# EI-CoreBioinformatics/portcullis

Hardware: AMD Instinct MI355X
Metric: junc_reads_per_sec (higher is better)
Workload: dtype int32; 1 GPU; BASELINE configs[2]: synthetic 199999998 paired-end 150-bp reads, 25 contigs of GRCh38 lengths (3088286401 bp), 249999 junctions, orientation FR; reads_total=199999998, junctions_total=249999, contigs=25, reads_rank0=199999998, pairs_rank0=66692850

## Files before the change

### portcullis_amd/csrc/pjb_api.hip

```cpp
#include "pjb_host.hip.h"
#include "pjb_kernels.hip.h"
#include "pjb_chain.hip.h"
#include "pjb_flight.hip.h"

extern "C" {

namespace {
std::mutex g_host_mu;
std::map<void *, size_t> g_host_registered;
}
void *pjb_host_alloc(size_t bytes) {
    if (bytes >= ((size_t)8 << 20)) {
        const size_t huge = (size_t)2 << 20, len = (bytes + huge - 1) & ~(huge - 1);
        void *p = mmap(nullptr, len, PROT_READ | PROT_WRITE, MAP_PRIVATE | MAP_ANONYMOUS, -1, 0);
        if (p != MAP_FAILED) {
            (void)madvise(p, len, MADV_HUGEPAGE);
            const size_t nt = std::min<size_t>(4, len >> 24);
            auto touch = [&](size_t t) {
                const size_t per = ((len / std::max<size_t>(nt, 1)) + huge - 1) & ~(huge - 1), a = std::min(len, per * t), b = std::min(len, a + per);
                for (size_t o = a; o < b; o += 4096) ((volatile uint8_t *)p)[o] = 0;
            };
            if (nt <= 1) touch(0);
            else {
                std::vector<std::thread> th;
                for (size_t t = 0; t < nt; t++) th.emplace_back(touch, t);
                for (auto &x : th) x.join();
            }
            if (hipHostRegister(p, len, hipHostRegisterDefault) == hipSuccess) {
                std::lock_guard<std::mutex> lk(g_host_mu);
                g_host_registered[p] = len;
                return p;
            }
            (void)hipGetLastError();
            munmap(p, len);
        }
    }
    void *p = nullptr;
    if (hipHostMalloc(&p, bytes ? bytes : 1, hipHostMallocDefault) != hipSuccess) return nullptr;
    return p;
}

void pjb_host_free(void *p) {
    if (!p) return;
    size_t len = 0;
    {
        std::lock_guard<std::mutex> lk(g_host_mu);
        auto it = g_host_registered.find(p);
        if (it != g_host_registered.end()) {
            len = it->second;
            g_host_registered.erase(it);
        }
    }
    if (len) {
        (void)hipHostUnregister(p);
        munmap(p, len);
    } else
        (void)hipHostFree(p);
}

int pjb_host_register(void *p, size_t bytes) {
    if (!p || !bytes) return PJB_ERR_ARG;
    if (hipHostRegister(p, bytes, hipHostRegisterDefault) != hipSuccess) {
        (void)hipGetLastError();
        return PJB_ERR_HIP;
    }
    return PJB_OK;
}
int pjb_host_unregister(void *p) {
    if (!p) return PJB_ERR_ARG;
    if (hipHostUnregister(p) != hipSuccess) {
        (void)hipGetLastError();
        return PJB_ERR_HIP;
    }
    return PJB_OK;
}

int pjb_device_count(void) {
    int n = 0;
    if (hipGetDeviceCount(&n) != hipSuccess) return 0;
    return n;
}

int pjb_create(pjb_ctx **out, const pjb_config *cfg) {
    if (!out || !cfg) return fail(nullptr, PJB_ERR_ARG, "pjb_create: null argument");
    *out = nullptr;
    if (cfg->abi_version != PJB_ABI_VERSION && cfg->abi_version != 3)
        return fail(nullptr, PJB_ERR_ARG, "pjb_create: ABI version %d, library is %d", cfg->abi_version, PJB_ABI_VERSION);
    if (cfg->orientation < PJB_OR_SE || cfg->orientation > PJB_OR_UNKNOWN)
        return fail(nullptr, PJB_ERR_ARG, "pjb_create: bad orientation %d", cfg->orientation);
    const bool ctrace = getenv("PJB_CREATE_TRACE") != nullptr;
    const auto ct0 = std::chrono::steady_clock::now();
    auto cmark = [&](const char *what) {
        if (ctrace) fprintf(stderr, "[pjb_create] %7.1f ms: %s\n", std::chrono::duration<double, std::milli>(std::chrono::steady_clock::now() - ct0).count(), what);
    };
    int n = 0;
    hipError_t e = hipGetDeviceCount(&n);
    cmark("hipGetDeviceCount");
    if (e != hipSuccess || n <= 0)
        return fail(nullptr, PJB_ERR_NO_DEVICE,
                    "no HIP device available (%s); the junc hot path has no CPU fallback",
                    e == hipSuccess ? "device count is 0" : hipGetErrorString(e));
    if (cfg->device < 0 || cfg->device >= n)
        return fail(nullptr, PJB_ERR_ARG, "pjb_create: device %d out of range (have %d)", cfg->device, n);
    e = hipSetDevice(cfg->device);
    if (e != hipSuccess) return fail(nullptr, PJB_ERR_HIP, "hipSetDevice(%d): %s", cfg->device, hipGetErrorString(e));
    hipDeviceProp_t prop;
    e = hipGetDeviceProperties(&prop, cfg->device);
    if (e != hipSuccess) return fail(nullptr, PJB_ERR_HIP, "hipGetDeviceProperties: %s", hipGetErrorString(e));
    cmark("hipSetDevice, hipGetDeviceProperties");
    const int n_cu = prop.multiProcessorCount;
    if (prop.warpSize != 64)
        return fail(nullptr, PJB_ERR_NO_DEVICE, "device %d (%s) is not a wave64 CDNA device", cfg->device, prop.gcnArchName);
    pjb_ctx *c = new (std::nothrow) pjb_ctx();
    if (!c) return fail(nullptr, PJB_ERR_NOMEM, "out of host memory");
    const int dev = cfg->device;
    auto attributes = [dev] {
        (void)hipSetDevice(dev);
        ingest_kernel_attributes();
        (void)hipFuncSetAttribute((const void *)rs_scatter<0, u64>, hipFuncAttributeMaxDynamicSharedMemorySize, (int)rs_scatter_lds_bytes(RS_MAX_BITS));
        (void)hipFuncSetAttribute((const void *)rs_scatter<0, u32>, hipFuncAttributeMaxDynamicSharedMemorySize, (int)rs_scatter_lds_bytes(RS_MAX_BITS, 4));
    };
    std::thread attr_thread(attributes);
    struct JoinAttr {
        std::thread &t;
        ~JoinAttr() {
            if (t.joinable()) t.join();
        }
    } join_attr{attr_thread};
    c->cfg = *cfg;
    memset(&c->timing, 0, sizeof c->timing);
    e = hipStreamCreateWithFlags(&c->stream, hipStreamNonBlocking);
    if (e != hipSuccess) {
        delete c;
        return fail(nullptr, PJB_ERR_HIP, "hipStreamCreate: %s", hipGetErrorString(e));
    }
    if (!(cfg->flags & PJB_FLAG_NO_CHAINS)) aux_streams(c);
    (void)hipEventCreateWithFlags(&c->ev_front, hipEventDisableTiming);
    c->scan_tiles = &c->b_scan_tiles;
    cmark("main streams");
    if (!(cfg->flags & PJB_FLAG_NO_CHAINS))
        for (int k = 0; k < 4 && k < PJB_MAX_QUEUED; k++) (void)slot_init(c, k);
    cmark("chain slots");
    c->inflate_lanes = std::max(1, n_cu) * (160 * 1024 / ingest_lds_bytes()) * 64;
    c->ktime = (cfg->flags & PJB_FLAG_KERNEL_TIMING) != 0;
    c->extra = (cfg->flags & PJB_FLAG_EXTRA) != 0;
    if (const char *s = getenv("PJB_K1_SERIAL")) c->k1_serial = atoi(s) != 0;
    if (const char *s = getenv("PJB_K1S_BLOCKS")) c->k1s_blocks_forced = std::max(0, std::min(atoi(s), (int)K1S_BLOCKS));
    if (const char *s = getenv("PJB_RADIX_BITS")) {
        int v = atoi(s);
        if (v >= 4 && v <= RS_MAX_BITS) c->radix_max_bits = v;
    }
    cmark("options");
    attr_thread.join();
    cmark("kernel attributes");
    *out = c;
    return PJB_OK;
}


void pjb_destroy(pjb_ctx *c) {
    if (!c) return;
    (void)hipSetDevice(c->cfg.device);
    (void)hipDeviceSynchronize();
    (void)exhume(c);
#ifdef K1E_PROF
    {
        unsigned long long h[16] = {0};
        (void)hipDeviceSynchronize();
        if (hipMemcpyFromSymbol(h, HIP_SYMBOL(pjb::g_k1e_prof), sizeof h) == hipSuccess) {
            unsigned long long tot = 0;
            for (int i = 0; i < 12; i++) tot += h[i];
            static const char *nm[12] = {"block start", "prologue", "shapes (wait ops)", "windows issue", "next records issue", "stage wait", "next ops issue", "compare+emit", "lists", "cand flush", "span of bases", "bases issue"};
            for (int i = 0; i < 12; i++) fprintf(stderr, "[k1e_prof] %-20s %6.2f %%  %llu\n", nm[i], tot ? 100.0 * (double)h[i] / (double)tot : 0.0, h[i]);
        }
    }
#endif
    while (!c->open.empty()) close_contig(c, c->open.begin()->first);
    extra_clear(c);
    for (auto &kv : c->filter_keys)
        if (kv.second.first) (void)hipFree(kv.second.first);
    c->filter_keys.clear();
    for (auto &g : c->contigs) free_contig(g);
    for (auto &b : c->genome_pool) release(b);
    c->genome_pool.clear();
    for (auto &sl : c->slab_pool)
        if (sl.p) (void)hipFree(sl.p);
    if (c->rows_pinned) (void)hipHostFree(c->rows_pinned);
    if (c->rows_table) (void)hipFree(c->rows_table);
    bam_stage_clear(c);
    for (int k = 0; k < PJB_MAX_QUEUED; k++) {
        CtlSlot &S = c->sl[k];
        if (S.pub) (void)hipHostFree(S.pub);
        if (S.batches_pinned) (void)hipHostFree(S.batches_pinned);
        for (auto &ev : S.ev)
            if (ev) (void)hipEventDestroy(ev);
        if (S.ev_rows) (void)hipEventDestroy(S.ev_rows);
        if (S.ev_done) (void)hipEventDestroy(S.ev_done);
        Buf *sb[] = {&S.x_q, &S.x_spos, &S.x_send, &S.x_gapoff, &S.x_zlist, &S.x_scnt, &S.x_codes, &S.cstats, &S.err, &S.gencount, &S.batches, &S.rows, &S.tile_cnt, &S.tile_stats, &S.splidx, &S.splpoff, &S.splrec, &S.tile_soff, &S.chunk_tile, &S.scan_parts, &S.members, &S.okey, &S.g,
                     &S.rec, &S.jidbam, &S.jkey, &S.total, &S.bitmap, &S.wrank, &S.pagecnt, &S.pagerank, &S.ends, &S.firstid,
                     &S.key[0], &S.key[1], &S.idx[0], &S.idx[1], &S.hist, &S.hist_scan, &S.hist_part, &S.bintotal, &S.scan_tiles, &S.jid, &S.seg, &S.runfirst,
                     &S.runstart, &S.ent, &S.entsum, &S.frag, &S.fragj, &S.masks, &S.acc, &S.ancl, &S.ancr, &S.genlist, &S.runs};
        for (Buf *b : sb) release(*b);
        hipEvent_t evs[] = {S.ev_k1, S.ev_xk1, S.ev_fork, S.ev_join, S.ev_fork2, S.ev_join2};
        for (hipEvent_t e : evs)
            if (e) (void)hipEventDestroy(e);
        if (S.main) (void)hipStreamDestroy(S.main);
        if (S.side) (void)hipStreamDestroy(S.side);
    }
    if (c->mirror_hdr) (void)hipHostFree(c->mirror_hdr);
    for (int k = 0; k < 2; k++) {
        if (c->stage[k]) (void)hipHostFree(c->stage[k]);
        if (c->stage_ev[k]) (void)hipEventDestroy(c->stage_ev[k]);
    }
    Buf *all[] = {&c->b_cursor, &c->b_scan_tiles, &c->b_hasx, &c->b_xtotal, &c->b_fasta_raw, &c->b_inf_comp, &c->b_inf_out, &c->b_inf_blocks, &c->b_inf_status, &c->b_inf_scratch, &c->b_inf_bitmap,
                  &c->b_bam_seg, &c->b_bam_rec, &c->b_bam_ctl, &c->f_pos, &c->f_cigoff, &c->f_cigar, &c->f_codes,
                  &c->x_pos, &c->x_endx, &c->x_q, &c->x_prefq, &c->x_ce, &c->x_bound, &c->x_de, &c->x_dropped, &c->x_zlist, &c->x_cnt,
                  &c->x_tabk, &c->x_tabc, &c->x_rs, &c->x_re, &c->x_rr, &c->x_tileoff, &c->x_xrall, &c->x_tab,
                  &c->b_dfl_in, &c->b_dfl_sym, &c->b_dfl_slots, &c->b_dfl_size, &c->b_dfl_off, &c->b_dfl_packed};
    for (Buf *b : all) release(*b);
    c->model.release_all();
    for (auto &ch : c->xarena.chunks) (void)hipFree(ch.p);
    if (c->xrows_pinned) (void)hipHostFree(c->xrows_pinned);
    for (auto &pool : c->pools)
        for (auto &ev : pool.ev) (void)hipEventDestroy(ev);
    if (c->ev_front) (void)hipEventDestroy(c->ev_front);
    if (c->stream3) (void)hipStreamDestroy(c->stream3);
    if (c->stream4) (void)hipStreamDestroy(c->stream4);
    (void)hipStreamDestroy(c->stream);
    delete c;
}

const char *pjb_last_error(const pjb_ctx *c) {
    if (!c) return g_create_error.c_str();
    return g_thread_error_ctx == c ? g_thread_error.c_str() : "";
}

int pjb_set_refs(pjb_ctx *c, int32_t n_refs, const int32_t *ref_len) {
    if (!c) return PJB_ERR_ARG;
    if (n_refs < 0 || (n_refs > 0 && !ref_len)) return fail(c, PJB_ERR_ARG, "pjb_set_refs: bad arguments");
    if (!c->open.empty()) return fail(c, PJB_ERR_STATE, "pjb_set_refs: contig %d is still open", c->open.begin()->first);
    for (auto &g : c->contigs) free_contig(g);
    c->ref_len.assign(ref_len, ref_len + n_refs);
    c->contigs.assign((size_t)n_refs, Contig());
    return PJB_OK;
}

static int upload_common(pjb_ctx *c, int32_t tid, uint8_t *d, int64_t len, bool owned, bool do_upper, size_t d_cap = 0, bool fasta_flag = false) {
    static const bool prof = getenv("PJB_PROFILE_HOST") != nullptr;
    const double t_up0 = wall_now();
    double t_alloc = 0;
    HIP_TRY(c, hipSetDevice(c->cfg.device));
    int rc = ensure(c, c->b_hasx, 4 * sizeof(int));
    if (rc) return rc;
    int *d_flags = (int *)c->b_hasx.p;
    HIP_TRY(c, hipMemsetAsync(d_flags, 0, 3 * sizeof(int), c->stream));
    if (len > 0) {
        const int64_t nthreads = (len + 15) / 16;
        const unsigned nblk = (unsigned)((nthreads + 255) / 256);
        hipLaunchKernelGGL(k0_upper, dim3(nblk), dim3(256), 0, c->stream, d, len, do_upper ? 1 : 0, d_flags + 0);
    }
    u32 *codes = nullptr;
    size_t codes_cap = 0;
    const int64_t n_words = (len + 7) / 8;
    static const bool no_seq2 = getenv("PJB_NO_SEQ2") && atoi(getenv("PJB_NO_SEQ2")) != 0;
    const size_t c2_at = ((size_t)(n_words + 2) + 3) & ~(size_t)3;
    const size_t c2_words = len > 0 && !no_seq2 ? (size_t)codes2_alloc_words(len) : 0;
    if (len > 0) {
        const double ta = wall_now();
        codes = (u32 *)genome_take(c->genome_pool, (c2_at + c2_words) * 4, codes_cap);
        t_alloc = wall_now() - ta;
        if (!codes) return fail(c, PJB_ERR_NOMEM, "hipMalloc(genome codes, %zu bytes) failed", (c2_at + c2_words) * 4);
        (void)hipMemsetAsync(codes + n_words, 0, 8, c->stream);
        hipLaunchKernelGGL(k0_encode, dim3((unsigned)((n_words + 255) / 256)), dim3(256), 0, c->stream, (const uint8_t *)d, len,
                           codes, n_words, d_flags + 1);
    }
    u32 *codes2 = nullptr;
    if (codes && c2_words) {
        codes2 = codes + c2_at;
        const int64_t n2w = codes2_words(len), nxw = gexc_words(len);
        (void)hipMemsetAsync(codes2 + n2w, 0, (size_t)K0_CODES2_PAD * 4, c->stream);
        (void)hipMemsetAsync(codes2 + n2w + K0_CODES2_PAD + nxw, 0, (size_t)K0_GEXC_PAD * 4, c->stream);
        hipLaunchKernelGGL(k0_encode2, dim3((unsigned)(((len + 63) / 64 + 255) / 256)), dim3(256), 0, c->stream, (const uint8_t *)d, len, codes2,
                           codes2 + n2w + K0_CODES2_PAD, d_flags + 2);
    }
    int flags[4] = {0, 0, 1, 0};
    HIP_TRY(c, hipMemcpyAsync(flags, d_flags, (fasta_flag ? 4 : 3) * sizeof(int), hipMemcpyDeviceToHost, c->stream));
    const double t_sync0 = wall_now();
    hipError_t se = hipStreamSynchronize(c->stream);
    if (se != hipSuccess) {
        if (codes) (void)hipFree(codes);
        return fail(c, PJB_ERR_HIP, "upload: %s", hipGetErrorString(se));
    }
    if (prof)
        fprintf(stderr, "[host profile] genome tid %d (%lld bases): codes allocation %.4f, launches %.4f, wait for the stream %.4f s\n", tid, (long long)len, t_alloc,
                t_sync0 - t_up0 - t_alloc, wall_now() - t_sync0);
    if (fasta_flag && flags[3]) {
        if (codes) (void)hipFree(codes);
        return 1;
    }
    const int hx = flags[0], exotic = flags[1], any_exc = codes2 ? flags[2] : 1;
    if (exotic && codes) {
        (void)hipFree(codes);
        codes = nullptr;
        codes2 = nullptr;
// ... 235 lines not shown
    return PJB_OK;
}

int pjb_set_row_mirror(pjb_ctx *c, void *device_buffer, int64_t cap_bytes) {
    if (!c) return PJB_ERR_ARG;
    if (device_buffer && cap_bytes < PJB_MIRROR_HEADER_BYTES) return fail(c, PJB_ERR_ARG, "set_row_mirror: buffer smaller than its header");
    if (c->n_fl) return fail(c, PJB_ERR_STATE, "set_row_mirror: target %d is still queued", c->fl[0].tid);
    c->mirror = (uint8_t *)device_buffer;
    c->mirror_cap = device_buffer ? (size_t)cap_bytes : 0;
    mirror_reset(c);
    if (c->mirror && !c->mirror_hdr) {
        HIP_TRY(c, hipSetDevice(c->cfg.device));
        HIP_TRY(c, hipHostMalloc((void **)&c->mirror_hdr, PJB_MIRROR_HEADER_BYTES, hipHostMallocDefault));
    }
    return PJB_OK;
}

int pjb_plan_groups(const int32_t *ref_len, const int32_t *tids, int32_t n_tids, int64_t max_bases, int32_t *group_of) {
    if (n_tids < 0 || (n_tids > 0 && (!ref_len || !tids || !group_of))) return PJB_ERR_ARG;
    if (max_bases <= 0) max_bases = (int64_t)1 << 30;
    auto span = [&](int32_t k) { return group_span(ref_len[tids[k]]); };
    auto plan = [&](int64_t cap) {
        int32_t g = 0, members = 0;
        int64_t tot = 0;
        for (int32_t k = 0; k < n_tids; k++) {
            const int64_t s = span(k);
            if (members && (tot + s > cap || members >= GROUP_MAX)) g++, members = 0, tot = 0;
            group_of[k] = g;
            members++;
            tot += s;
        }
        return n_tids ? g + 1 : 0;
    };
    for (int32_t k = 0; k < n_tids; k++)
        if (tids[k] < 0) return PJB_ERR_ARG;
    int32_t n = plan(max_bases);
    if (n == 1 && n_tids > 1) {
        int64_t total = 0;
        for (int32_t k = 0; k < n_tids; k++) total += span(k);
        if (total > 600000000) n = plan((int64_t)((double)total * 0.55));
    }
    return n;
}

int pjb_merge_rows(const void *gathered, int32_t n_ranks, int64_t slot_stride_bytes, pjb_junction_row *rows_out, int64_t cap_rows, int64_t *n_rows,
                   pjb_region_result *totals) {
    if (n_rows) *n_rows = 0;
    if (!gathered || n_ranks < 1 || slot_stride_bytes < PJB_MIRROR_HEADER_BYTES || !n_rows || !totals || cap_rows < 0 || (cap_rows > 0 && !rows_out))
        return PJB_ERR_ARG;
    struct Run {
        int32_t refid;
        const pjb_junction_row *first;
        int64_t n;
    };
    std::vector<Run> runs;
    pjb_region_result T;
    memset(&T, 0, sizeof T);
    T.min_len = INT32_MAX;
    int64_t total = 0;
    for (int32_t r = 0; r < n_ranks; r++) {
        const uint8_t *slot = (const uint8_t *)gathered + (size_t)r * (size_t)slot_stride_bytes;
        int64_t h[6];
        memcpy(h, slot, sizeof h);
        if (h[0] < 0 || h[0] > (slot_stride_bytes - PJB_MIRROR_HEADER_BYTES) / (int64_t)sizeof(pjb_junction_row)) return PJB_ERR_ARG;
        T.spliced += (uint64_t)h[1];
        T.unspliced += (uint64_t)h[2];
        T.sum_len += (uint64_t)h[3];
        T.min_len = std::min<int32_t>(T.min_len, (int32_t)std::min<int64_t>(h[4], INT32_MAX));
        T.max_len = std::max<int32_t>(T.max_len, (int32_t)h[5]);
        const pjb_junction_row *rows = (const pjb_junction_row *)(slot + PJB_MIRROR_HEADER_BYTES);
        for (int64_t i = 0; i < h[0];) {
            int64_t j = i + 1;
            while (j < h[0] && rows[j].refid == rows[i].refid) j++;
            runs.push_back(Run{rows[i].refid, rows + i, j - i});
            i = j;
        }
        total += h[0];
    }
    T.n_reads = (int64_t)(T.spliced + T.unspliced);
    T.n_junctions = total;
    *totals = T;
    *n_rows = total;
    if (total > cap_rows) return PJB_ERR_ARG;
    std::stable_sort(runs.begin(), runs.end(), [](const Run &a, const Run &b) { return a.refid < b.refid; });
    pjb_junction_row *out = rows_out;
    for (const Run &u : runs) {
        memcpy(out, u.first, (size_t)u.n * sizeof(pjb_junction_row));
        out += u.n;
    }
    return PJB_OK;
}

int pjb_clear_rows(pjb_ctx *c) {
    if (!c) return PJB_ERR_ARG;
    if (c->n_fl) return fail(c, PJB_ERR_STATE, "clear_rows: target %d is still queued", c->fl[0].tid);
    (void)rows_sync(c);
    c->rows_n = 0;
    (void)exhume(c);
    mirror_reset(c);
    if (c->extra) {
        (void)hipSetDevice(c->cfg.device);
        (void)hipStreamSynchronize(c->stream);
        extra_clear(c);
    }
    return PJB_OK;
}

int pjb_get_kernel_timing(const pjb_ctx *c, pjb_kernel_time *out, int32_t cap, int32_t *n) {
    if (!c || !n) return PJB_ERR_ARG;
    *n = (int32_t)c->knames.size();
    for (int32_t i = 0; out && i < cap && i < *n; i++) {
        memset(&out[i], 0, sizeof out[i]);
        strncpy(out[i].name, c->knames[(size_t)i].c_str(), sizeof(out[i].name) - 1);
        out[i].launches = c->kcount[(size_t)i];
        out[i].total_ms = c->kms[(size_t)i];
    }
    return PJB_OK;
}

int pjb_select_timed_kernels(pjb_ctx *c, const char *comma_separated_names) {
    if (!c) return PJB_ERR_ARG;
    c->ktime_only.clear();
    std::string s = comma_separated_names ? comma_separated_names : "";
    size_t a = 0;
    while (a < s.size()) {
        size_t b = s.find(',', a);
        if (b == std::string::npos) b = s.size();
        if (b > a) c->ktime_only.push_back(s.substr(a, b - a));
        a = b + 1;
    }
    return PJB_OK;
}

int pjb_reset_kernel_timing(pjb_ctx *c) {
    if (!c) return PJB_ERR_ARG;
    std::fill(c->kcount.begin(), c->kcount.end(), 0);
    std::fill(c->kms.begin(), c->kms.end(), 0.0);
    return PJB_OK;
}

int pjb_set_option(pjb_ctx *c, const char *name, int64_t value) {
    if (!c || !name) return PJB_ERR_ARG;
    if (c->n_fl) return fail(c, PJB_ERR_STATE, "set_option: target %d is still queued", c->fl[0].tid);
    const std::string n = name;
    if (n == "overlap") c->side_stream = value != 0;
    else if (n == "dense_ids") c->dense_ids = value != 0;
    else if (n == "extra_dense") c->extra_dense_only = value != 0;
    else if (n == "sort_floor") c->sort_floor = (u32)std::max<int64_t>(1, std::min<int64_t>(value, 1 << 30));
    else if (n == "window_skip") c->window_skip = value != 0;
    else if (n == "run_sort") c->run_sort = value != 0;
    else if (n == "run_window") {
        if (value < 0 || value > (int64_t)RUN_W) return fail(c, PJB_ERR_ARG, "set_option: run_window takes 0 (the default, %u) to %u", RUN_W, RUN_W);
        c->run_window = (u32)value;
    } else if (n == "grow_batch") {
        if (value < 0 || value > 32768) return fail(c, PJB_ERR_ARG, "set_option: grow_batch takes 0 (the default: what the pool holds) to 32768 trees");
        c->model.grow_batch = (u32)value;
    } else if (n == "knn_chunk") {
        if (value < 0 || value > (1 << 22)) return fail(c, PJB_ERR_ARG, "set_option: knn_chunk takes 0 (the default: sized to fill the chip) to %d base rows", 1 << 22);
        c->model.knn_chunk = (u32)value;
    } else if (n == "list_cap") c->list_cap_forced = (u32)std::max<int64_t>(0, std::min<int64_t>(value, 1 << 30));
    else return fail(c, PJB_ERR_ARG, "set_option: unknown option '%s'", name);
    return PJB_OK;
}

int pjb_get_timing(const pjb_ctx *c, pjb_timing *out) {
    if (!c || !out) return PJB_ERR_ARG;
    if (c->cfg.abi_version >= 4) *out = c->timing;
    else memcpy(out, &c->timing, offsetof(pjb_timing, repeats));
    return PJB_OK;
}

}
```

### portcullis_amd/csrc/pjb_chain.hip.h

```cpp
#pragma once

constexpr unsigned K6_BLOCKS = 128;

static size_t rows_upper_bound(const pjb_ctx *c) {
    size_t n = c->rows_n;
    for (int k = 0; k < c->n_fl; k++)
        if (c->fl[k].queued) n += c->fl[k].lim.junc_limit;
    return n;
}

static void wait_flight(pjb_ctx *c, Flight &f) {
    if (f.queued) (void)hipEventSynchronize(c->sl[f.slot].ev_done);
}

static int rows_table_reserve(pjb_ctx *c, Flight &f, u32 JL) {
    size_t old = rows_upper_bound(c);
    if (old + JL <= c->rows_cap) return PJB_OK;
    for (int k = 0; k < c->n_fl; k++)
        if (c->fl[k].queued && &c->fl[k] != &f) wait_flight(c, c->fl[k]);
    int rc = rows_sync(c);
    if (rc) return rc;
    old = std::min(old, c->rows_cap);
    const size_t ncap = std::max<size_t>((old + JL) * 3 / 2, 1024);
    pjb_junction_row *nd = nullptr;
    hipError_t e = hipMalloc((void **)&nd, ncap * sizeof(pjb_junction_row));
    if (e != hipSuccess) return fail(c, PJB_ERR_NOMEM, "hipMalloc(row table): %s", hipGetErrorString(e));
    if (old) {
        HIP_TRY(c, hipMemcpyAsync(nd, c->rows_table, old * sizeof(pjb_junction_row), hipMemcpyDeviceToDevice, c->stream4));
        HIP_TRY(c, hipStreamSynchronize(c->stream4));
    }
    if (c->rows_table) bury(c, c->rows_table);
    c->rows_table = nd;
    c->rows_cap = ncap;
    return PJB_OK;
}

struct Chain {
    pjb_ctx *c;
    Flight &f;
    CtlSlot &S;
    hipStream_t st, service;
    GroupTab GT;
    bool group, fast_codes, any_x, stage_events, xk1, dense_moved, entropy_forked;
    int n_members;
    int32_t ref_len;
    KeyFmt kf;
    u32 PL, JL, SL;
    u32 n_tiles, pair_blocks, slots_lim, n_slices_lim, gen_cap, pack_nn;
    size_t n_words;
    int64_t row_base, mirror_base;
    u32 rs_tiles, run_cap, ro_tiles, plan_tiles;
    bool run_route, first_hist_done;
    int sort_bits, n_pass, pass_bits[16], cur;
    RunOut ro;
    u64 *ro_total, *ro_key[2];
    u32 *run_dest, *ro_idx[2];
    u64 *d_err;
    ContigStats *d_cs;
    const u32 *d_P, *d_J, *d_slots;
    MemberStats *d_members;
    u32 *d_member_junc, *d_tile_lo, *d_gen_cnt;
    Pairs pr;
};

struct ChainScope {
    pjb_ctx *c;
    hipStream_t stream = c->stream;
    Buf *scan_tiles = c->scan_tiles;
    int pool = c->cur_pool;
    ~ChainScope() {
        c->stream = stream;
        c->scan_tiles = scan_tiles;
        c->cur_pool = pool;
    }
};

#define STAGE_EVENT(k)                                                     \
    do {                                                                   \
        if (ch.stage_events) HIP_TRY(c, hipEventRecord(S.ev[k], ch.st));   \
    } while (0)

template <typename Fn>
static int chain_fork(Chain &ch, hipEvent_t ev_fork, hipEvent_t ev_join, bool &forked, Fn fn) {
    pjb_ctx *c = ch.c;
    if (!c->side_stream) return fn(ch);
    HIP_TRY(c, hipEventRecord(ev_fork, ch.st));
    HIP_TRY(c, hipStreamWaitEvent(ch.S.side, ev_fork, 0));
    c->stream = ch.S.side;
    forked = true;
    const int rc = fn(ch);
    c->stream = ch.st;
    if (rc) return rc;
    HIP_TRY(c, hipEventRecord(ev_join, ch.S.side));
    return PJB_OK;
}

static int chain_plan(Chain &ch) {
    pjb_ctx *c = ch.c;
    Flight &f = ch.f;
    const ContigLimits &lim = f.lim;
    ch.service = c->stream;
    ch.st = c->side_stream ? ch.S.main : c->stream;
    ch.n_tiles = f.n_tiles;
    ch.n_members = (int)f.tids.size();
    ch.group = ch.n_members > 1;
    ch.ref_len = ch.group ? (int32_t)f.vlen : c->ref_len[(size_t)f.tid];
    GroupTab &GT = ch.GT;
    memset(&GT, 0, sizeof GT);
    GT.n = ch.n_members;
    bool all_codes = true;
    ch.any_x = false;
    for (int m = 0; m < ch.n_members; m++) {
        const Contig &g = c->contigs[(size_t)f.tids[(size_t)m]];
        GT.voff[m] = f.voff[(size_t)m];
        GT.len[m] = (int32_t)g.len;
        GT.tid[m] = f.tids[(size_t)m];
        GT.d[m] = g.d;
        GT.codes[m] = g.codes;
        GT.codes2[m] = g.codes2;
        if (g.any_exc) GT.exc_members |= 1u << m;
        all_codes = all_codes && g.codes != nullptr;
        ch.any_x = ch.any_x || g.has_x;
    }
    ch.fast_codes = all_codes && !ch.any_x;
    ch.kf = lim.kf;
    const u32 PL = ch.PL = lim.pair_limit, JL = ch.JL = lim.junc_limit;
    ch.SL = lim.sort_limit && lim.sort_limit < JL ? lim.sort_limit : JL;
    bool ahead = false;
    for (int k = 0; k < c->n_fl; k++) ahead |= c->fl[k].queued && &c->fl[k] != &f;
    ch.row_base = ahead ? -1 : (int64_t)c->rows_n;
    ch.mirror_base = ahead ? -1 : (int64_t)c->mirror_rows;
    ch.pair_blocks = std::max<u32>(1, (PL + 255) / 256);
    ch.gen_cap = lim.list_cap ? lim.list_cap : (c->list_cap_forced ? c->list_cap_forced : gen_list_cap(PL));
    ch.pack_nn = (u64)ch.n_tiles * K1_TILE < (1ull << 28) ? 1u : 0u;
    ch.slots_lim = JL + (PL + 63) / 64 + 1;
    ch.n_slices_lim = (PL + 63) / 64 + 1;
    ch.n_words = ((size_t)std::max(ch.ref_len, 1) + 63) / 64;
    ch.stage_events = c->ktime && c->ktime_only.empty();
    ch.xk1 = c->extra && !c->extra_dense_only && !ch.group && !f.x_k1 && !f.x_pre;
    ch.rs_tiles = std::max<u32>(1, (PL + RS_TILE - 1) / RS_TILE);
    ch.run_route = lim.dense && lim.run_sort;
    ch.run_cap = (u32)std::min<u64>((u64)PL / 8 + 64ull * ch.rs_tiles, 0xfff00000ull);
    ch.ro_tiles = (ch.run_cap + RS_TILE - 1) / RS_TILE;
    if (ch.run_route) {
        ch.ro.cap = ch.run_cap;
        ch.ro.window = c->run_window ? std::min<u32>(c->run_window, RUN_W) : RUN_W;
        ch.ro.tile_bits = std::max(1, bits_of((uint64_t)ch.rs_tiles));
    }
    ch.sort_bits = lim.dense ? std::max(1, bits_of((uint64_t)ch.SL)) + (ch.run_route ? ch.ro.tile_bits : 0) : ch.kf.total_bits;
    ch.plan_tiles = ch.run_route ? ch.ro_tiles : ch.rs_tiles;
    ch.first_hist_done = lim.dense && !ch.run_route;
    ch.n_pass = std::max(1, (ch.sort_bits + c->radix_max_bits - 1) / c->radix_max_bits);
    for (int p = 0; p < ch.n_pass; p++) ch.pass_bits[p] = ch.sort_bits / ch.n_pass + (p < ch.sort_bits % ch.n_pass ? 1 : 0);
    return PJB_OK;
}

static RunOut run_carve(Chain &ch, int &rc) {
    pjb_ctx *c = ch.c;
    CtlSlot &S = ch.S;
    RunOut ro = ch.ro;
    auto al = [](size_t b) { return (b + 255) & ~(size_t)255; };
    const u32 rs_tiles = ch.rs_tiles, run_cap = ch.run_cap;
    const size_t slack = (size_t)run_cap + RS_TILE;
    const size_t at_tf = 256, at_tn = at_tf + al((size_t)rs_tiles * 4), at_key = at_tn + al((size_t)rs_tiles * 4), at_cnt = at_key + al(slack * 8),
                 at_dest = at_cnt + al((size_t)run_cap * 4), at_k0 = at_dest + al((size_t)run_cap * 4), at_k1 = at_k0 + al(slack * 8),
                 at_i0 = at_k1 + al(slack * 8), at_i1 = at_i0 + al(slack * 4), at_end = at_i1 + al(slack * 4);
    if ((rc = ensure(c, S.runs, at_end))) return ro;
    uint8_t *b = (uint8_t *)S.runs.p;
    ro.n_runs = (u32 *)b;
    ch.ro_total = (u64 *)(b + 8);
    ro.tile_first = (u32 *)(b + at_tf);
    ro.tile_n = (u32 *)(b + at_tn);
    ro.key = (u64 *)(b + at_key);
    ro.cnt = (u32 *)(b + at_cnt);
    ch.run_dest = (u32 *)(b + at_dest);
    ch.ro_key[0] = (u64 *)(b + at_k0);
    ch.ro_key[1] = (u64 *)(b + at_k1);
    ch.ro_idx[0] = (u32 *)(b + at_i0);
    ch.ro_idx[1] = (u32 *)(b + at_i1);
    return ro;
}

static int chain_room(Chain &ch) {
    pjb_ctx *c = ch.c;
    Flight &f = ch.f;
    CtlSlot &S = ch.S;
    const std::vector<DevBatch> &batches = f.batches;
    const u32 PL = ch.PL, JL = ch.JL, n_tiles = ch.n_tiles;
    const size_t n_words = ch.n_words, N = (size_t)f.n_reads;
    const u32 plan_tiles = ch.plan_tiles;
    const int dbits = ch.pass_bits[0];
    const bool dense = f.lim.dense;
    int rc;
    if (batches.size() + 2 > S.batches_pinned_cap) {
        if (S.batches_pinned) (void)hipHostFree(S.batches_pinned);
        S.batches_pinned = nullptr;
        S.batches_pinned_cap = 0;
        const size_t cap = std::max<size_t>(batches.size() * 2 + 2, 16);
        HIP_TRY(c, hipHostMalloc((void **)&S.batches_pinned, cap * sizeof(DevBatch), hipHostMallocDefault));
        S.batches_pinned_cap = cap;
    }
    memcpy(S.batches_pinned, batches.data(), batches.size() * sizeof(DevBatch));
    const struct { Buf *b; size_t bytes; bool whole; } once[] = {
        {&S.scan_parts, sizeof(ScanPart) * K1S_BLOCKS, false},
        {&c->b_cursor, sizeof(RowCursor), false},
        {&S.members, GROUP_MAX * sizeof(MemberStats) + GROUP_MAX * 4 + (GROUP_MAX + 1) * 4, true},
    };
    for (const auto &o : once) {
        if (o.b->p) continue;
        if ((rc = ensure(c, *o.b, o.bytes))) return rc;
        HIP_TRY(c, hipMemset(o.b->p, 0, o.whole ? o.b->cap : o.bytes));
        HIP_TRY(c, hipStreamSynchronize(nullptr));
    }
    const void *was[3] = {S.bitmap.p, S.ends.p, S.pagecnt.p};
    const struct { Buf *b; size_t bytes; bool on = true; } room[] = {
        {&S.batches, batches.size() * sizeof(DevBatch)},
        {&S.cstats, sizeof(ContigStats)},
        {&S.err, 8},
        {&S.tile_cnt, (size_t)n_tiles * 4},
        {&S.tile_stats, (size_t)n_tiles * sizeof(TileStats)},
        {&S.tile_soff, ((size_t)n_tiles + 1) * 4},
        {&S.chunk_tile, ((size_t)n_tiles * (K1_TILE / 256) + 4) * 4},
        {&S.splidx, (size_t)n_tiles * K1_TILE * 4},
        {&S.splpoff, (size_t)n_tiles * K1_TILE * 4},
        {&S.splrec, (size_t)n_tiles * K1_TILE * 16},
        {&S.total, 8},
        {&S.okey, ((size_t)PL + RS_TILE) * 8},
        {&S.key[0], ((size_t)PL + RS_TILE) * 8},
        {&S.key[1], ((size_t)PL + RS_TILE) * 8},
        {&S.idx[0], ((size_t)PL + RS_TILE) * 4},
        {&S.idx[1], ((size_t)PL + RS_TILE) * 4},
        {&S.rec, ((size_t)PL + 1) * sizeof(PairRec)},
        {&S.jid, (size_t)PL * 4 + 16},
        {&S.jidbam, ((size_t)PL + RS_TILE) * 4},
        {&S.g, (size_t)PL * 4 + 16, c->extra},
        {&S.seg, ((size_t)PL + 1) * 4},
        {&S.runfirst, ((size_t)PL + 1) * 4},
        {&S.runstart, ((size_t)PL + 1) * 4},
        {&S.ent, (size_t)PL * 8 + 16},
        {&S.genlist, (size_t)ch.gen_cap * GEN_SHARDS * 8 * 3},
        {&S.gencount, GEN_SHARDS * GEN_CNT_STRIDE * 4},
        {&S.frag, (size_t)ch.slots_lim * F_WORDS * 4},
        {&S.fragj, (size_t)ch.slots_lim * 4},
        {&S.acc, (size_t)JL * F_WORDS * 4 + 16},
        {&S.ancl, (size_t)JL * 4 + 16},
        {&S.ancr, (size_t)JL * 4 + 16},
        {&S.jkey, (size_t)JL * 8 + 16},
        {&S.rows, (size_t)JL * sizeof(pjb_junction_row) + 16},
        {&S.entsum, (size_t)JL * 8 + 16},
        {&S.bitmap, n_words * 8 + 16, dense},
        {&S.wrank, n_words * 4 + 16, dense},
        {&S.pagecnt, ((n_words >> KD_PAGE_SHIFT) + 1) * 4 + 16, dense},
        {&S.pagerank, ((n_words >> KD_PAGE_SHIFT) + 1) * 4 + 16, dense},
        {&S.ends, (size_t)JL * DENSE_ENDS * 4 + 32, dense},
        {&S.firstid, (size_t)JL * 4 + 16, dense},
        {&S.masks, (size_t)ch.n_slices_lim * 8 * 2 + (size_t)ch.n_slices_lim * 4, dense},
        {&S.hist, (size_t)plan_tiles * (1u << dbits) * 4},
        {&S.hist_scan, (size_t)plan_tiles * (1u << dbits) * 4},
        {&S.bintotal, (size_t)4 << dbits},
        {&S.hist_part, (size_t)((plan_tiles + RSP_TILES - 1) / RSP_TILES) * (1u << dbits) * 4},
        {&S.x_q, N + 16, ch.xk1},
        {&S.x_spos, N * 4 + 16, ch.xk1},
        {&S.x_send, N * 4 + 16, ch.xk1},
        {&S.x_zlist, (size_t)X_ZCAP * 8, ch.xk1},
        {&S.x_scnt, X_SCNT_BYTES, ch.xk1},
    };
    for (const auto &r : room)
        if (r.on && (rc = ensure(c, *r.b, r.bytes))) return rc;
    ch.dense_moved = was[0] != S.bitmap.p || was[1] != S.ends.p || was[2] != S.pagecnt.p;
    if (ch.run_route) {
        ch.ro = run_carve(ch, rc);
        if (rc) return rc;
    }
    if ((rc = rows_table_reserve(c, f, JL))) return rc;
    if (!S.pub) {
        HIP_TRY(c, hipHostMalloc((void **)&S.pub, PUB_BYTES, hipHostMallocMapped | hipHostMallocPortable));
        void *dp = nullptr;
        if (hipHostGetDevicePointer(&dp, S.pub, 0) != hipSuccess || !dp) return fail(c, PJB_ERR_HIP, "hipHostGetDevicePointer(control block) failed");
        S.pub_dev = (uint8_t *)dp;
    }
    ch.d_members = (MemberStats *)S.members.p;
    ch.d_member_junc = (u32 *)(ch.d_members + GROUP_MAX);
    ch.d_tile_lo = ch.d_member_junc + GROUP_MAX;
    ch.d_err = (u64 *)S.err.p;
    ch.d_cs = (ContigStats *)S.cstats.p;
    ch.d_P = &ch.d_cs->P;
    ch.d_J = &ch.d_cs->J;
    ch.d_slots = &ch.d_cs->n_slots;
    ch.d_gen_cnt = (u32 *)S.gencount.p;
    ch.pr.key = (u64 *)S.okey.p;
    ch.pr.rec = (PairRec *)S.rec.p;
    ch.pr.g = c->extra ? (u32 *)S.g.p : (u32 *)nullptr;
    return PJB_OK;
}

static int chain_front(Chain &ch) {
    pjb_ctx *c = ch.c;
    Flight &f = ch.f;
    CtlSlot &S = ch.S;
    const hipStream_t st = ch.st;
    const size_t n_batches = f.batches.size();
    bool on_service = false;
    for (int32_t t : f.tids) {
        auto oit = c->open.find(t);
        on_service = on_service || (oit != c->open.end() && oit->second.on_main_stream);
    }
    if (st != ch.service && on_service) {
        HIP_TRY(c, hipEventRecord(c->ev_front, ch.service));
        HIP_TRY(c, hipStreamWaitEvent(st, c->ev_front, 0));
    }
    HIP_TRY(c, hipMemcpyAsync(S.batches.p, S.batches_pinned, n_batches * sizeof(DevBatch), hipMemcpyHostToDevice, st));
    if (ch.group) {
        u32 *h_lo = (u32 *)(S.batches_pinned + n_batches);
        for (int m = 0; m <= ch.n_members; m++) h_lo[m] = f.tile_lo[(size_t)m];
        HIP_TRY(c, hipMemcpyAsync(ch.d_tile_lo, h_lo, (size_t)(ch.n_members + 1) * 4, hipMemcpyHostToDevice, st));
    }
    if (!S.at_rest) {
        HIP_TRY(c, hipMemsetAsync(S.err.p, 0xff, 8, st));
        HIP_TRY(c, hipMemsetAsync(S.gencount.p, 0, GEN_SHARDS * GEN_CNT_STRIDE * 4, st));
        HIP_TRY(c, hipMemsetAsync(ch.d_member_junc, 0, GROUP_MAX * 4, st));
    }
    S.at_rest = false;
    HIP_TRY(c, hipEventRecord(S.ev[0], st));
    if (f.lim.dense) {
        if (!S.dense_at_rest || ch.dense_moved) {
            HIP_TRY(c, hipMemsetAsync(S.bitmap.p, 0, S.bitmap.cap, st));
            HIP_TRY(c, hipMemsetAsync(S.pagecnt.p, 0, S.pagecnt.cap, st));
            HIP_TRY(c, hipMemsetAsync(S.ends.p, 0xff, S.ends.cap, st));
        }
        S.dense_at_rest = false;
    }
    f.pr = ch.pr;
    return PJB_OK;
}

static int chain_k1(Chain &ch) {
    pjb_ctx *c = ch.c;
    Flight &f = ch.f;
    CtlSlot &S = ch.S;
    const std::vector<DevBatch> &batches = f.batches;
    const hipStream_t st = ch.st;
    const GroupTab &GT = ch.GT;
    const KeyFmt kf = ch.kf;
    const u32 n_tiles = ch.n_tiles;
    const bool k1_late = getenv("PJB_K1_SERIAL_LATE") != nullptr;
    XOut xo = {nullptr, nullptr, nullptr, nullptr, 0, nullptr};
    if (ch.xk1) {
        const size_t N = (size_t)f.n_reads;
        HIP_TRY(c, hipMemsetAsync((uint8_t *)S.x_q.p + N, 0, 1, c->stream));
        HIP_TRY(c, hipMemsetAsync(S.x_scnt.p, 0, sizeof(SparseCounters) + sizeof(ExtraCounters), c->stream));
        xo = XOut{(int32_t *)S.x_spos.p, (int32_t *)S.x_send.p, (uint8_t *)S.x_q.p, (u32 *)S.x_zlist.p, X_ZCAP, (SparseCounters *)S.x_scnt.p};
    }
    if (c->k1_serial && c->last_k1_ev) HIP_TRY(c, hipStreamWaitEvent(st, c->last_k1_ev, 0));
    if (ch.xk1)
        LAUNCH(c, "k1_count", k1_count<true>, dim3(n_tiles), dim3(K1C_T), (const DevBatch *)S.batches.p, (int)batches.size(), (u32 *)S.tile_cnt.p, (TileStats *)S.tile_stats.p,
               (u32 *)S.splidx.p, (u32 *)S.splpoff.p, (uint4 *)S.splrec.p, ch.d_err, GT, 0, xo);
    else
        LAUNCH(c, "k1_count", k1_count<false>, dim3(n_tiles), dim3(K1C_T), (const DevBatch *)S.batches.p, (int)batches.size(), (u32 *)S.tile_cnt.p, (TileStats *)S.tile_stats.p,
               (u32 *)S.splidx.p, (u32 *)S.splpoff.p, (uint4 *)S.splrec.p, ch.d_err, GT, ch.group ? 1 : 0, xo);
    if (ch.xk1) {
        HIP_TRY(c, hipEventRecord(S.ev_xk1, c->stream));
        f.x_k1 = true;
    }
    LAUNCH(c, "k1_scan_tiles", k1_scan_tiles, dim3(c->k1s_blocks_forced ? (u32)c->k1s_blocks_forced : k1s_blocks(n_tiles)), dim3(K1S_THREADS), (u32 *)S.tile_cnt.p, (const TileStats *)S.tile_stats.p,
           n_tiles, ch.d_cs, ch.PL, kf, ch.group ? INT32_MAX - 1 : ch.ref_len, (const u64 *)nullptr, (u32 *)S.tile_soff.p, (u32 *)S.chunk_tile.p,
           (ScanPart *)S.scan_parts.p, ++S.scan_epoch, c->window_skip ? 1u : 0u);
    EmitLists el;
    el.cand = f.lim.dense ? (u64 *)S.key[1].p : (u64 *)nullptr;
    el.bitmap = f.lim.dense ? (u64 *)S.bitmap.p : (u64 *)nullptr;
    el.page_cnt = f.lim.dense ? (u32 *)S.pagecnt.p : (u32 *)nullptr;
    el.cand_anc = (u64 *)S.ent.p;
    el.gen_list = (u64 *)S.genlist.p;
    el.gen_cnt = ch.d_gen_cnt;
    el.gen_cap = ch.gen_cap;
    el.pack_nn = ch.pack_nn;
    for (size_t b0 = 0; b0 < batches.size(); b0 += K1E_MAXB) {
        const size_t nb = std::min<size_t>(K1E_MAXB, batches.size() - b0);
        u64 reads = 0;
        for (size_t bi = b0; bi < b0 + nb; bi++) reads += (u64)batches[bi].n;
        const u32 nt = (u32)std::min<u64>((reads + K1_TILE - 1) / K1_TILE + nb, 0x7fffffffu);
        static const u32 tiles_per_block = getenv("PJB_K1E_TILES") ? (u32)std::max(1, atoi(getenv("PJB_K1E_TILES"))) : 8u;
        const u32 grid = std::max<u32>(1, std::min<u32>(nt, std::max<u32>(1024, nt / tiles_per_block)));
        LAUNCH(c, "k1_emit", k1_emit, dim3(grid), dim3(256), (const DevBatch *)S.batches.p + b0, (int)nb, n_tiles, (const u32 *)S.tile_cnt.p,
               (const u32 *)S.tile_soff.p, (const u32 *)S.chunk_tile.p, (const u32 *)S.splidx.p, (const u32 *)S.splpoff.p, (const uint4 *)S.splrec.p, ch.pr, el, kf,
               GT, ch.fast_codes ? 1 : 0, (int)c->cfg.orientation, ch.d_err, ch.d_cs);
    }
    if (c->k1_serial && !k1_late) {
        HIP_TRY(c, hipEventRecord(S.ev_k1, st));
        c->last_k1_ev = S.ev_k1;
    }
    if (ch.group)
        LAUNCH(c, "kg_member_stats", kg_member_stats, dim3((unsigned)ch.n_members), dim3(256), (const u32 *)S.tile_cnt.p, (const TileStats *)S.tile_stats.p,
               (const u32 *)ch.d_tile_lo, ch.n_members, ch.d_members, n_tiles, (const ContigStats *)ch.d_cs);
    LAUNCH(c, "k1_generic", k1_generic, dim3(std::min<u32>(std::max<u32>(1, (u32)(((u64)ch.gen_cap * GEN_SHARDS + K1E_T - 1) / K1E_T)), 1536u )), dim3(K1E_T),
           (const DevBatch *)S.batches.p, (int)batches.size(), (const u32 *)S.splidx.p, (const uint4 *)S.splrec.p, ch.pr, el, kf, GT, ch.fast_codes ? 1 : 0,
           (int)c->cfg.orientation, ch.d_err, ch.d_cs);
    if (c->k1_serial && k1_late) {
        HIP_TRY(c, hipEventRecord(S.ev_k1, st));
        c->last_k1_ev = S.ev_k1;
    }
    STAGE_EVENT(1);
    return PJB_OK;
}

static int chain_k4b(Chain &ch) {
    pjb_ctx *c = ch.c;
    CtlSlot &S = ch.S;
    const u32 gen_grid = std::min<u32>(2 * (u32)(((u64)ch.gen_cap * GEN_SHARDS + 255) / 256), 2560u);
    LAUNCH(c, "k4b_generic", k4b_generic, dim3(gen_grid), dim3(256), (const u64 *)S.genlist.p, (const u32 *)ch.d_gen_cnt, ch.gen_cap, (const u64 *)ch.pr.key,
           ch.pr.rec, (const u32 *)S.jidbam.p, ch.kf, (const DevBatch *)S.batches.p, (int)ch.f.batches.size(), (const int32_t *)S.ancl.p, (const int32_t *)S.ancr.p,
           ch.GT, ch.any_x ? 1 : 0, ch.any_x ? 0 : 1, ch.d_err, (const ContigStats *)ch.d_cs, ch.pack_nn, (const u32 *)S.splidx.p, (const uint4 *)S.splrec.p);
    return PJB_OK;
}

static int chain_k2d(Chain &ch) {
    pjb_ctx *c = ch.c;
    Flight &f = ch.f;
    CtlSlot &S = ch.S;
    if (!f.lim.dense) return PJB_OK;
    const KeyFmt kf = ch.kf;
    const u32 JL = ch.JL;
    const size_t n_words = ch.n_words;
    int rc;
    const u32 cand_blocks = std::min<u32>(ch.pair_blocks, 1024u);
    const u64 *okey = (const u64 *)ch.pr.key;
    u64 *cand = (u64 *)S.key[1].p;
    const u32 n_pages = (u32)((n_words + ((size_t)1 << KD_PAGE_SHIFT) - 1) >> KD_PAGE_SHIFT);
    if ((rc = run_scan(c, "kd_rank", ArrU32Fn{(const u32 *)S.pagecnt.p}, ExclusiveU32Sink{(u32 *)S.pagerank.p}, (u64)n_pages, (u64 *)S.total.p)))
        return rc;
    LAUNCH(c, "kd_rank_pages", kd_rank_pages, dim3((n_pages + 3) / 4), dim3(256), (const u64 *)S.bitmap.p, (const u32 *)S.pagecnt.p, (const u32 *)S.pagerank.p,
           (u32 *)S.wrank.p, n_pages, (u32)n_words);
    u32 *cand_rank = (u32 *)S.idx[1].p;
    LAUNCH(c, "kd_ends", kd_ends, dim3(cand_blocks), dim3(256), (const u64 *)cand, kf, (const u64 *)S.bitmap.p, (const u32 *)S.wrank.p, JL,
           (u32 *)S.ends.p, cand_rank, ch.d_cs);
    if ((rc = run_scan(c, "kd_first", EndsCountFn{(const u32 *)S.ends.p}, FirstIdSink{(u32 *)S.firstid.p, (int32_t *)S.ancl.p, (int32_t *)S.ancr.p},
                       (u64)JL, (u64 *)S.total.p)))
        return rc;
    LAUNCH(c, "kd_table", kd_table, dim3(cand_blocks), dim3(256), (const u64 *)cand, (const u64 *)S.ent.p, (const u32 *)cand_rank, kf, JL,
           (const u32 *)S.ends.p, (const u32 *)S.firstid.p, (const u64 *)S.total.p, (u64 *)S.jkey.p, (int32_t *)S.ancl.p, (int32_t *)S.ancr.p, ch.d_cs,
           (const u32 *)ch.d_gen_cnt, ch.gen_cap, ch.SL, ch.ro.n_runs);
    LAUNCH(c, "kd_assign", kd_assign, dim3(ch.rs_tiles), dim3(256), okey, ch.d_P, kf, (const u64 *)S.bitmap.p, (const u32 *)S.wrank.p,
           (const u32 *)S.ends.p, (const u32 *)S.firstid.p, JL, (const u64 *)S.total.p, (u32 *)S.jidbam.p, (u32 *)S.acc.p, (const u64 *)S.jkey.p,
           (const int32_t *)S.ancl.p, (const int32_t *)S.ancr.p, ch.d_err, ch.d_cs, ch.run_route ? 0 : ch.pass_bits[0], (u32 *)S.hist.p, ch.ro);
    if ((rc = chain_fork(ch, S.ev_fork, S.ev_join, f.forked, chain_k4b))) return rc;
    LAUNCH(c, "kd_reset", kd_reset, dim3(cand_blocks), dim3(256), (const u64 *)cand, (const u32 *)cand_rank, kf, JL, (const ContigStats *)ch.d_cs,
           (u64 *)S.bitmap.p, (u32 *)S.ends.p, (u32 *)S.pagecnt.p);
    S.dense_at_rest = true;
    return PJB_OK;
}

static const char *const rs_names[4] = {"rs_hist", "rs_panel_sums", "rs_panel_scan", "rs_scatter"};
static const char *const ro_names[6] = {"ro_hist", "ro_panel_sums", "ro_panel_scan", "ro_scatter", "ro_offsets", "rs_place"};

template <typename K>
static int sort_pass(Chain &ch, const void *kin_v, void *kout_v, const u32 *vin, u32 *vout, int shift, int bits, const u32 *d_n, u32 tiles,
                     const char *const *names) {
    pjb_ctx *c = ch.c;
    CtlSlot &S = ch.S;
    const K *kin = (const K *)kin_v;
    K *kout = (K *)kout_v;
    if (!(shift == 0 && ch.first_hist_done))
        LAUNCH(c, names[0], rs_hist<K>, dim3(tiles), dim3(256), kin, d_n, shift, bits, (u32 *)S.hist.p, tiles);
    {
        const u32 nb = 1u << bits, n_panels = (tiles + RSP_TILES - 1) / RSP_TILES;
        LAUNCH(c, names[1], rs_panel_sums, dim3(n_panels, (nb + 255) / 256), dim3(256), (const u32 *)S.hist.p, tiles, nb, (u32 *)S.hist_part.p);
        LAUNCH(c, names[2], rs_panel_scan, dim3(n_panels, (nb + 255) / 256), dim3(256), (const u32 *)S.hist.p, (const u32 *)S.hist_part.p, tiles, nb,
               (u32 *)S.hist_scan.p, (u32 *)S.bintotal.p);
    }
#define RS_SCATTER(B)                                                                                                                          \
    LAUNCH_LDS(c, names[3], (rs_scatter<B, K>), dim3(tiles), dim3(256), rs_scatter_lds_bytes(bits, sizeof(K)), kin, vin, kout, vout, d_n, \
               shift, bits, (const u32 *)S.hist_scan.p, (const u32 *)S.bintotal.p, tiles)
    switch (bits) {
    case 9: RS_SCATTER(9); break;
    case 10: RS_SCATTER(10); break;
    case 11: RS_SCATTER(11); break;
    default: RS_SCATTER(0); break;
    }
#undef RS_SCATTER
    return PJB_OK;
}

static int chain_sort(Chain &ch) {
    pjb_ctx *c = ch.c;
    Flight &f = ch.f;
    CtlSlot &S = ch.S;
    const RunOut &ro = ch.ro;
    int rc = PJB_OK, cur = 0, shift = 0;
    for (int p = 0; p < ch.n_pass; p++) {
        const int bits = ch.pass_bits[p];
        if (bits <= 0) break;
        if (ch.run_route) {
            rc = sort_pass<u64>(ch, p == 0 ? (const void *)ro.key : (const void *)ch.ro_key[cur], ch.ro_key[cur ^ 1], p == 0 ? nullptr : (const u32 *)ch.ro_idx[cur],
                                ch.ro_idx[cur ^ 1], shift, bits, (const u32 *)ro.n_runs, ch.ro_tiles, ro_names);
        } else {
            const u32 *vin = p == 0 ? nullptr : (const u32 *)S.idx[cur].p;
            u32 *vout = (u32 *)S.idx[cur ^ 1].p;
            if (f.lim.dense) rc = sort_pass<u32>(ch, p == 0 ? S.jidbam.p : S.key[cur].p, S.key[cur ^ 1].p, vin, vout, shift, bits, ch.d_P, ch.rs_tiles, rs_names);
            else rc = sort_pass<u64>(ch, p == 0 ? S.okey.p : S.key[cur].p, S.key[cur ^ 1].p, vin, vout, shift, bits, ch.d_P, ch.rs_tiles, rs_names);
        }
        if (rc) return rc;
        cur ^= 1;
        shift += bits;
    }
    f.n_pass = ch.n_pass;
    if (ch.run_route) {
        const u32 *order = ch.ro_idx[cur];
        if ((rc = run_scan(c, ro_names[4], RunCountFn{(const u32 *)ro.cnt, order}, RunDestSink{ch.run_dest, order}, (u64)ch.run_cap, ch.ro_total, (const u32 *)ro.n_runs)))
            return rc;
        cur = 1;
        LAUNCH(c, ro_names[5], rs_place, dim3(ch.rs_tiles), dim3(256), (const u32 *)S.jidbam.p, ch.d_P, (const u64 *)ro.key, (const u32 *)ch.run_dest,
               (const u32 *)ro.tile_first, (const u32 *)ro.tile_n, ch.run_cap, ro.tile_bits, (u32 *)S.key[cur].p, (u32 *)S.idx[cur].p);
        f.n_pass = 1;
    }
    ch.cur = cur;
    f.sidx = (const u32 *)S.idx[cur].p;
    f.jid_sorted = f.lim.dense ? (const u32 *)S.key[cur].p : (const u32 *)S.jid.p;
    STAGE_EVENT(2);
    return PJB_OK;
}

static int chain_entropy(Chain &ch) {
    pjb_ctx *c = ch.c;
    CtlSlot &S = ch.S;
    LAUNCH(c, "k5_entropy_sum", k5_entropy_sum, dim3(std::max<u32>(1, (ch.JL + 15) / 16)), dim3(256), (const u32 *)S.seg.p, (const u32 *)S.runfirst.p,
           (const u32 *)S.runstart.p, ch.d_J, (double *)S.entsum.p);
    return PJB_OK;
}

#ifdef PJB_DEBUG_LAUNCH
static void debug_sort_check(Chain &ch) {
    Flight &f = ch.f;
    CtlSlot &S = ch.S;
    const int cur = ch.cur;
    fprintf(stderr, "[k4_pairs] tid %d PL %u JL %u slots_lim %u n_slices_lim %u frag cap %zu fragj cap %zu masks cap %zu rec cap %zu idx cap %zu key cap %zu jkey cap %zu cur %d n_pass %d\n",
            f.tid, ch.PL, ch.JL, ch.slots_lim, ch.n_slices_lim, S.frag.cap, S.fragj.cap, S.masks.cap, S.rec.cap, S.idx[cur].cap, S.key[cur].cap, S.jkey.cap, cur, f.n_pass);
    ContigStats hcs;
    (void)hipDeviceSynchronize();
    (void)hipMemcpy(&hcs, ch.d_cs, sizeof hcs, hipMemcpyDeviceToHost);
    u64 htot = 0;
    (void)hipMemcpy(&htot, S.total.p, 8, hipMemcpyDeviceToHost);
    fprintf(stderr, "[k4_pairs] cs: P %u n_pairs %llu J %u n_junc %u n_slots %u n_slices %u n_cand %u overflow %u R %u total %llu slot %d attempt %d\n", hcs.P,
            (unsigned long long)hcs.n_pairs, hcs.J, hcs.n_junc, hcs.n_slots, hcs.n_slices, hcs.n_cand, hcs.overflow, hcs.R, (unsigned long long)htot, f.slot, f.attempt);
    std::vector<u32> hs(hcs.P), hj(hcs.P), hb(hcs.P);
    (void)hipMemcpy(hs.data(), f.sidx, (size_t)hcs.P * 4, hipMemcpyDeviceToHost);
    (void)hipMemcpy(hj.data(), f.jid_sorted, (size_t)hcs.P * 4, hipMemcpyDeviceToHost);
    (void)hipMemcpy(hb.data(), S.jidbam.p, (size_t)hcs.P * 4, hipMemcpyDeviceToHost);
    std::vector<char> seen(hcs.P, 0);
    size_t bad_idx = 0, dup = 0, bad_order = 0, bad_in = 0, mism = 0;
    long first_bad = -1;
    for (size_t i = 0; i < hcs.P; i++) {
        if (hb[i] >= hcs.J) bad_in++;
        if (hs[i] >= hcs.P) {
            bad_idx++;
            if (first_bad < 0) first_bad = (long)i;
            continue;
        }
        if (seen[hs[i]]) dup++;
        seen[hs[i]] = 1;
        if (hj[i] != hb[hs[i]]) mism++;
        if (i && hj[i] < hj[i - 1]) bad_order++;
    }
    fprintf(stderr, "[k4_pairs] sort check: %zu indices out of range (first at %ld), %zu duplicates, %zu order breaks, %zu key/index mismatches, %zu input ids >= J\n", bad_idx,
            first_bad, dup, bad_order, mism, bad_in);
}
#endif

static int chain_runs_dense(Chain &ch) {
    pjb_ctx *c = ch.c;
    Flight &f = ch.f;
    CtlSlot &S = ch.S;
    const u32 n_slices_lim = ch.n_slices_lim, pair_blocks = ch.pair_blocks;
    int rc;
    u64 *head_mask = (u64 *)S.masks.p, *run_mask = head_mask + n_slices_lim;
    u32 *run_base = (u32 *)(run_mask + n_slices_lim);
    STAGE_EVENT(3);
    STAGE_EVENT(4);
    if (f.forked) HIP_TRY(c, hipStreamWaitEvent(ch.st, S.ev_join, 0));
#ifdef PJB_DEBUG_LAUNCH
    debug_sort_check(ch);
#endif
    LAUNCH(c, "k4_pairs", k4_pairs, dim3(pair_blocks), dim3(256), f.sidx, f.jid_sorted, (const PairRec *)ch.pr.rec, (const u64 *)S.jkey.p, ch.kf, ch.d_P,
           (u32 *)S.frag.p, (int32_t *)S.fragj.p, head_mask, run_mask, (const ContigStats *)ch.d_cs, ch.d_err);
    if ((rc = run_scan(c, "k2_runs", Popc64Fn{(const u64 *)run_mask}, ExclusiveU32Sink{run_base}, (u64)n_slices_lim, (u64 *)S.total.p, &ch.d_cs->n_slices)))
        return rc;
    LAUNCH(c, "k2_expand", k2_expand, dim3((pair_blocks + K2E_PER - 1) / K2E_PER), dim3(256), f.jid_sorted, (const u64 *)head_mask, (const u64 *)run_mask, (const u32 *)run_base,
           (const u64 *)S.total.p, (u32 *)S.seg.p, (u32 *)S.runfirst.p, (u32 *)S.runstart.p, ch.d_cs);
    STAGE_EVENT(5);
    return chain_fork(ch, S.ev_fork2, S.ev_join2, ch.entropy_forked, chain_entropy);
}

static int chain_runs_keys(Chain &ch) {
    pjb_ctx *c = ch.c;
    Flight &f = ch.f;
    CtlSlot &S = ch.S;
    const u32 JL = ch.JL, pair_blocks = ch.pair_blocks;
    int rc;
    const u64 *skey = (const u64 *)S.key[ch.cur].p;
    HeadFn hf{skey, f.sidx, (const PairRec *)ch.pr.rec};
    HeadSink hs{(u32 *)S.jid.p, (u32 *)S.seg.p, (u32 *)S.runfirst.p, (u32 *)S.runstart.p, skey, (u64 *)S.jkey.p, JL};
    if ((rc = run_scan(c, "k2_heads", hf, hs, (u64)ch.PL, (u64 *)S.total.p, ch.d_P))) return rc;
    LAUNCH(c, "k2_close", k2_close, dim3(1), dim3(1), (u64 *)S.total.p, (u32 *)S.seg.p, (u32 *)S.runfirst.p,
           (u32 *)S.runstart.p, ch.d_cs, JL, (const u32 *)ch.d_gen_cnt, ch.gen_cap);
    STAGE_EVENT(3);
    if ((rc = chain_fork(ch, S.ev_fork2, S.ev_join2, ch.entropy_forked, chain_entropy))) return rc;
    LAUNCH(c, "kf_init", kf_init, dim3(std::max<u32>(1, std::min<u32>((JL * F_WORDS + 255) / 256, 4096))), dim3(256), (u32 *)S.acc.p, ch.d_J, (int32_t *)S.ancl.p,
           (int32_t *)S.ancr.p);
    LAUNCH(c, "kf_anchors", kf_anchors, dim3(pair_blocks), dim3(256), f.sidx, (const u32 *)S.jid.p, (const PairRec *)ch.pr.rec, ch.d_P, (u32 *)S.jidbam.p,
           (int32_t *)S.ancl.p, (int32_t *)S.ancr.p);
    if ((rc = chain_k4b(ch))) return rc;
    STAGE_EVENT(4);
    LAUNCH(c, "k4_pairs", k4_pairs, dim3(pair_blocks), dim3(256), f.sidx, f.jid_sorted, (const PairRec *)ch.pr.rec, (const u64 *)S.jkey.p, ch.kf, ch.d_P,
           (u32 *)S.frag.p, (int32_t *)S.fragj.p, (u64 *)nullptr, (u64 *)nullptr, (const ContigStats *)ch.d_cs, ch.d_err);
    STAGE_EVENT(5);
    return PJB_OK;
}

static int chain_rows(Chain &ch) {
    pjb_ctx *c = ch.c;
    Flight &f = ch.f;
    CtlSlot &S = ch.S;
    const hipStream_t st = ch.st;
    const u32 JL = ch.JL;
    LAUNCH(c, "k5_frag_reduce", k5_frag_reduce, dim3((ch.slots_lim + 4 * FRAG_SLOTS_PER_WAVE - 1) / (4 * FRAG_SLOTS_PER_WAVE)), dim3(256),
           (const u32 *)S.frag.p, (const int32_t *)S.fragj.p, ch.d_slots, (u32 *)S.acc.p);
    if (ch.entropy_forked) HIP_TRY(c, hipStreamWaitEvent(st, S.ev_join2, 0));
    LAUNCH(c, "k5_finalize", k5_finalize, dim3(std::max<u32>(1, (JL + 255) / 256)), dim3(256), (const u64 *)S.jkey.p, (const u32 *)S.seg.p,
           (const u32 *)S.runfirst.p, (const u32 *)S.runstart.p, (const u32 *)S.acc.p,
           (const int32_t *)S.ancl.p, (const int32_t *)S.ancr.p, ch.kf, ch.GT, ch.d_J, (const double *)S.entsum.p, (pjb_junction_row *)S.rows.p, ch.d_err,
           ch.d_member_junc);
    STAGE_EVENT(6);
    u64 *mirror_table = nullptr;
    u32 mirror_room = 0;
    if (c->mirror && c->mirror_cap >= PJB_MIRROR_HEADER_BYTES) {
        mirror_table = (u64 *)(c->mirror + PJB_MIRROR_HEADER_BYTES);
        mirror_room = (u32)std::min<size_t>((c->mirror_cap - PJB_MIRROR_HEADER_BYTES) / sizeof(pjb_junction_row), 0xffffffffu);
    }
    const hipStream_t rows_stream = c->side_stream ? c->stream3 : st;
    if (rows_stream != st) {
        HIP_TRY(c, hipEventRecord(S.ev_rows, st));
        HIP_TRY(c, hipStreamWaitEvent(rows_stream, S.ev_rows, 0));
    }
    {
        ChainScope scope{c};
        c->stream = rows_stream;
        LAUNCH(c, "k6_rows_out", k6_rows_out, dim3(K6_BLOCKS), dim3(256), (const u64 *)S.rows.p, (const ContigStats *)ch.d_cs,
               (u64 *)c->rows_table, ch.row_base, ch.mirror_base, (RowCursor *)c->b_cursor.p, mirror_table, mirror_room, ch.d_err, ch.d_gen_cnt, S.pub_dev,
               (const MemberStats *)ch.d_members, ch.d_member_junc, ch.n_members);
    }
    S.at_rest = true;
    HIP_TRY(c, hipEventRecord(S.ev[7], rows_stream));
    HIP_TRY(c, hipEventRecord(S.ev_done, rows_stream));
    f.queued = true;
    return PJB_OK;
}
#undef STAGE_EVENT

static int queue_contig(pjb_ctx *c, Flight &f) {
    Chain ch{c, f, c->sl[f.slot]};
    int rc = chain_plan(ch);
    ChainScope scope{c};
    c->stream = ch.st;
    c->scan_tiles = &ch.S.scan_tiles;
    c->cur_pool = c->cur_slot = f.slot;
    ev_drop(c, f.slot);
    if (rc || (rc = chain_room(ch)) || (rc = chain_front(ch)) || (rc = chain_k1(ch)) || (rc = chain_k2d(ch)) || (rc = chain_sort(ch)) ||
        (rc = f.lim.dense ? chain_runs_dense(ch) : chain_runs_keys(ch)))
        return rc;
    return chain_rows(ch);
}
```

### portcullis_amd/csrc/pjb_device.hip.h

```cpp
#pragma once

#include <hip/hip_runtime.h>
#include <stdint.h>

#include "../../include/portcullis_amd.h"

namespace pjb {

typedef unsigned long long u64;
typedef unsigned int u32;

struct DevBatch {
    const int32_t *pos;
    const uint16_t *flag;
    const uint8_t *mapq;
    const uint8_t *xs;
    const int32_t *l_qseq;
    const int32_t *mtid;
    const int32_t *mpos;
    const uint32_t *cig_off;
    const uint32_t *cigar;
    const uint32_t *seq_off;
    const uint8_t *seq4;
    const u64 *name_hash;
    int64_t n;
    uint32_t base;
    uint32_t tile_base;
    int32_t prev_pos;
    int32_t member;
    const int32_t *prev_pos_ptr;
    const uint32_t *seq2;
    const uint32_t *seq_exc;
};

__device__ inline void set_error(u64 *err, u32 ordinal, int code) {
    atomicMin(err, ((u64)ordinal << 8) | (u64)(u32)(-code));
}

struct TileStats {
    u32 spliced, unspliced;
    u64 sum_len;
    int32_t min_len, max_len;
    int32_t max_end;
    int32_t max_nlen;
    int32_t min_pos;
    u32 max_span;
};
static_assert(sizeof(TileStats) == 40, "TileStats layout");

enum : u32 { OVF_PAIRS = 1u, OVF_KEYFMT = 2u, OVF_JUNC = 4u, OVF_DENSE = 8u, OVF_LISTS = 16u, OVF_RUNS = 64u  };
struct ContigStats {
    u64 spliced, unspliced, sum_len;
    int32_t min_len, max_len;
    int32_t max_end, max_nlen, min_pos;
    u32 n_tiles;
    u64 n_pairs;
    u64 err;
    u32 n_junc, n_runs;
    u32 P;
    u32 J, R;
    u32 n_slots;
    u32 overflow;
    u32 n_cand;
    u32 n_slices;
    u32 list_need;
    u32 max_span;
};
static_assert(sizeof(ContigStats) == 112, "ContigStats layout");
__device__ __forceinline__ bool window_reach(u32 blk, u32 nl_prev, u32 nl_next, u32 B) {
    const u32 l = __builtin_elementwise_add_sat(blk, nl_prev), r = __builtin_elementwise_add_sat(__builtin_elementwise_add_sat(blk, nl_next), 1u);
    return l <= B || r <= B;
}

struct __attribute__((aligned(16))) PairRec {
    u64 aux;
    int32_t lstart;
    int32_t rend;
    int32_t pos;
    int32_t aend;
    u32 meta;
    u32 updown;
};
static_assert(sizeof(PairRec) == 32, "PairRec is one 32-byte sector");
struct Pairs {
    u64 *key;
    PairRec *rec;
    u32 *g;
};
__device__ __forceinline__ void rec_store(PairRec *dst, const PairRec &r) {
    uint4 *q = reinterpret_cast<uint4 *>(dst);
    q[0] = make_uint4((u32)r.aux, (u32)(r.aux >> 32), (u32)r.lstart, (u32)r.rend);
    q[1] = make_uint4((u32)r.pos, (u32)r.aend, r.meta, r.updown);
}
__device__ __forceinline__ PairRec rec_load(const PairRec *src) {
    const uint4 *q = reinterpret_cast<const uint4 *>(src);
    const uint4 a = q[0], b = q[1];
    PairRec r;
    r.aux = (u64)a.x | ((u64)a.y << 32);
    r.lstart = (int32_t)a.z;
    r.rend = (int32_t)a.w;
    r.pos = (int32_t)b.x;
    r.aend = (int32_t)b.y;
    r.meta = b.z;
    r.updown = b.w;
    return r;
}

enum : u32 {
    META_CAT_MASK = 3u,
    META_MULTI = 1u << 2,
    META_XS_SHIFT = 3,
    META_UM = 1u << 5,
    META_BPP = 1u << 6,
    META_PPP = 1u << 7,
    META_REL = 1u << 8,
    META_SIMPLE = 1u << 9,
};
__device__ __forceinline__ u64 pack_res(u32 minMatch, u32 mmes, u32 mis) {
    return (u64)(minMatch & 0xfffffu) | ((u64)(mmes & 0xfffffu) << 20) | ((u64)mis << 40);
}
constexpr u32 RES_FIELD_MAX = 0xfffffu;

constexpr int GROUP_MAX = 32;
constexpr int32_t GROUP_GAP = 4096;
struct GroupTab {
    int32_t n;
    int32_t voff[GROUP_MAX];
    int32_t len[GROUP_MAX];
    int32_t tid[GROUP_MAX];
    const uint8_t *d[GROUP_MAX];
    const u32 *codes[GROUP_MAX];
    const u32 *codes2[GROUP_MAX];
    u32 exc_members;
};
struct Member {
    int32_t idx, voff, len, tid;
    const uint8_t *d;
    const u32 *codes;
};
__device__ __forceinline__ Member member_of(const GroupTab &T, int32_t vpos) {
    int m = 0;
    if (T.n > 1) {
#pragma unroll
        for (int s = GROUP_MAX / 2; s >= 1; s >>= 1)
            if (m + s < T.n && T.voff[m + s] <= vpos) m += s;
    }
    Member M;
    M.idx = m;
    M.voff = T.voff[m];
    M.len = T.len[m];
    M.tid = T.tid[m];
    M.d = T.d[m];
    M.codes = T.codes[m];
    return M;
}
struct MemberStats {
    u64 spliced, unspliced, sum_len, n_pairs;
    int32_t min_len, max_len;
    u32 n_junc, _pad;
};

struct KeyFmt {
    int raw;
    int lbits;
    int total_bits;
};
__device__ __host__ inline u64 make_key(const KeyFmt &f, int32_t istart, int32_t iend) {
    if (f.raw) return ((u64)(u32)istart << 32) | (u64)(u32)iend;
    return ((u64)(u32)istart << f.lbits) | (u64)(u32)(iend - istart + 1);
}
__device__ __host__ inline void unpack_key(const KeyFmt &f, u64 k, int32_t &istart, int32_t &iend) {
    if (f.raw) {
        istart = (int32_t)(u32)(k >> 32);
        iend = (int32_t)(u32)k;
    } else {
        istart = (int32_t)(u32)(k >> f.lbits);
        iend = istart + (int32_t)(u32)(k & ((1ull << f.lbits) - 1)) - 1;
    }
}

__device__ __forceinline__ bool op_consumes_ref(u32 op) { return (0x18Du >> op) & 1u; }
__device__ __forceinline__ bool op_consumes_query(u32 op) { return (0x193u >> op) & 1u; }
enum : u32 { OP_M = 0, OP_I = 1, OP_D = 2, OP_N = 3, OP_S = 4, OP_H = 5, OP_P = 6, OP_EQ = 7, OP_X = 8 };

__device__ __forceinline__ int lane_id() { return threadIdx.x & 63; }
__device__ __forceinline__ void lds_barrier() {
    asm volatile("s_waitcnt lgkmcnt(0)" ::: "memory");
    __builtin_amdgcn_s_barrier();
    asm volatile("" ::: "memory");
}

template <class T>
__device__ __forceinline__ T gload(const T *p) {
    T v;
    __builtin_memcpy(&v, (const __attribute__((address_space(1))) void *)p, sizeof(T));
    return v;
}
#define PJB_GLOBAL __attribute__((address_space(1)))
template <class T>
__device__ __forceinline__ const PJB_GLOBAL T *as_global(const T *p) {
    return (const PJB_GLOBAL T *)p;
}
template <class T, class U>
__device__ __forceinline__ T gload_as(const PJB_GLOBAL U *p) {
    T v;
    __builtin_memcpy(&v, (const PJB_GLOBAL void *)p, sizeof(T));
    return v;
}
struct GBatch {
    const PJB_GLOBAL int32_t *pos;
    const PJB_GLOBAL uint16_t *flag;
    const PJB_GLOBAL uint8_t *mapq;
    const PJB_GLOBAL uint8_t *xs;
    const PJB_GLOBAL int32_t *l_qseq;
    const PJB_GLOBAL int32_t *mtid;
    const PJB_GLOBAL int32_t *mpos;
    const PJB_GLOBAL uint32_t *cig_off;
    const PJB_GLOBAL uint32_t *cigar;
    const PJB_GLOBAL uint32_t *seq_off;
    const PJB_GLOBAL uint8_t *seq4;
    int64_t n;
    uint32_t base, tile_base;
    int32_t prev_pos, member;
    const PJB_GLOBAL int32_t *prev_pos_ptr;
    const PJB_GLOBAL uint32_t *seq2, *seq_exc;
};
#define PJB_CONSTANT __attribute__((address_space(4)))
__device__ __forceinline__ GBatch load_batch(const DevBatch *d) {
    const PJB_CONSTANT DevBatch *g = (const PJB_CONSTANT DevBatch *)d;
    GBatch b;
    b.pos = as_global(g->pos);
    b.flag = as_global(g->flag);
    b.mapq = as_global(g->mapq);
    b.xs = as_global(g->xs);
    b.l_qseq = as_global(g->l_qseq);
    b.mtid = as_global(g->mtid);
    b.mpos = as_global(g->mpos);
    b.cig_off = as_global(g->cig_off);
    b.cigar = as_global(g->cigar);
    b.seq_off = as_global(g->seq_off);
    b.seq4 = as_global(g->seq4);
    b.n = g->n;
    b.base = g->base;
    b.tile_base = g->tile_base;
    b.prev_pos = g->prev_pos;
    b.member = g->member;
    b.prev_pos_ptr = as_global(g->prev_pos_ptr);
    b.seq2 = as_global(g->seq2);
    b.seq_exc = as_global(g->seq_exc);
    return b;
}
struct __attribute__((packed, aligned(4))) Words4 {
    u32 x, y, z, w;
};

template <typename T>
__device__ __forceinline__ T wave_sum(T v) {
#pragma unroll
    for (int o = 32; o > 0; o >>= 1) v += __shfl_down(v, o, 64);
    return v;
}
template <typename T>
__device__ __forceinline__ T wave_max(T v) {
#pragma unroll
    for (int o = 32; o > 0; o >>= 1) {
        T t = __shfl_down(v, o, 64);
        v = t > v ? t : v;
    }
    return v;
}
template <typename T>
__device__ __forceinline__ T wave_min(T v) {
#pragma unroll
    for (int o = 32; o > 0; o >>= 1) {
        T t = __shfl_down(v, o, 64);
        v = t < v ? t : v;
    }
    return v;
}
template <typename T>
__device__ __forceinline__ T wave_iscan(T v) {
    int l = lane_id();
#pragma unroll
    for (int o = 1; o < 64; o <<= 1) {
        T t = __shfl_up(v, o, 64);
        if (l >= o) v += t;
    }
    return v;
}

template <int CTRL, int ROW_MASK>
__device__ __forceinline__ u32 dpp_move(u32 ident, u32 v) {
    return (u32)__builtin_amdgcn_update_dpp((int)ident, (int)v, CTRL, ROW_MASK, 0xf, false);
}
struct DppAdd {
    static constexpr u32 ident = 0u;
    __device__ __forceinline__ static u32 op(u32 a, u32 b) { return a + b; }
};
struct DppMax {
    static constexpr u32 ident = 0u;
    __device__ __forceinline__ static u32 op(u32 a, u32 b) { return a > b ? a : b; }
};
struct DppMin {
    static constexpr u32 ident = 0xffffffffu;
    __device__ __forceinline__ static u32 op(u32 a, u32 b) { return a < b ? a : b; }
};
template <typename Op>
__device__ __forceinline__ u32 wave_total(u32 v) {
    v = Op::op(v, dpp_move<0xB1, 0xf>(Op::ident, v));
    v = Op::op(v, dpp_move<0x4E, 0xf>(Op::ident, v));
    v = Op::op(v, dpp_move<0x141, 0xf>(Op::ident, v));
    v = Op::op(v, dpp_move<0x140, 0xf>(Op::ident, v));
    v = Op::op(v, dpp_move<0x142, 0xa>(Op::ident, v));
    v = Op::op(v, dpp_move<0x143, 0xc>(Op::ident, v));
    return (u32)__builtin_amdgcn_readlane((int)v, 63);
}

template <typename T>
__device__ __forceinline__ T block_escan_256(T v, T *smem, T *total) {
    T inc = wave_iscan(v);
    int w = threadIdx.x >> 6, l = lane_id();
    __syncthreads();
    if (l == 63) smem[w] = inc;
    __syncthreads();
    T base = 0, tot = 0;
#pragma unroll
    for (int i = 0; i < 4; i++) {
        T s = smem[i];
        if (i < w) base += s;
        tot += s;
    }
    *total = tot;
    return base + inc - v;
}

template <int NW, typename T, bool LDS_ONLY = false>
__device__ __forceinline__ T block_escan(T v, T *smem, T *total) {
    T inc = wave_iscan(v);
    if constexpr (NW == 1) {
        *total = __shfl(inc, 63, 64);
        return inc - v;
    } else {
        int w = threadIdx.x >> 6, l = lane_id();
        if constexpr (LDS_ONLY) lds_barrier();
        else __syncthreads();
        if (l == 63) smem[w] = inc;
        if constexpr (LDS_ONLY) lds_barrier();
        else __syncthreads();
        T base = 0, tot = 0;
#pragma unroll
        for (int i = 0; i < NW; i++) {
            T s = smem[i];
            if (i < w) base += s;
            tot += s;
        }
        *total = tot;
        return base + inc - v;
    }
}

template <typename T, typename OP>
__device__ __forceinline__ T seg_reduce_to_head(T v, u32 segkey, OP op) {
    const int l = lane_id();
#pragma unroll
    for (int o = 1; o < 64; o <<= 1) {
        T t = __shfl_down(v, o, 64);
        u32 k = __shfl_down(segkey, o, 64);
        if (l + o < 64 && k == segkey) v = op(v, t);
    }
    return v;
}
struct OpMin { template <typename T> __device__ T operator()(T a, T b) const { return a < b ? a : b; } };
struct OpMax { template <typename T> __device__ T operator()(T a, T b) const { return a > b ? a : b; } };
struct OpAdd { template <typename T> __device__ T operator()(T a, T b) const { return a + b; } };

constexpr int SCAN_TILE = 2048;

template <typename F>
__global__ __launch_bounds__(256) void scan_reduce_kernel(F f, u64 n, u64 *tile_sums, const u32 *np) {
    __shared__ u64 sm[4];
    if (np) {
        const u64 d = *np;
        n = d < n ? d : n;
    }
    u64 base = (u64)blockIdx.x * SCAN_TILE;
    u64 s = 0;
#pragma unroll
    for (int k = 0; k < 8; k++) {
        u64 i = base + (u64)k * 256 + threadIdx.x;
        if (i < n) s += f(i);
    }
    s = wave_sum(s);
    if (lane_id() == 0) sm[threadIdx.x >> 6] = s;
    __syncthreads();
    if (threadIdx.x == 0) tile_sums[blockIdx.x] = sm[0] + sm[1] + sm[2] + sm[3];
}

template <int UNUSED = 0>
__global__ __launch_bounds__(1024) void scan_tiles_kernel(u64 *tile_sums, u32 n_tiles, u64 *total) {
    __shared__ u64 wsum[16];
    __shared__ u64 carry_s;
    if (threadIdx.x == 0) carry_s = 0;
    __syncthreads();
    for (u32 base = 0; base < n_tiles; base += 1024) {
        u32 i = base + threadIdx.x;
        u64 v = i < n_tiles ? tile_sums[i] : 0;
        u64 inc = wave_iscan(v);
        int w = threadIdx.x >> 6;
        if (lane_id() == 63) wsum[w] = inc;
        __syncthreads();
        u64 wb = 0, tot = 0;
        for (int k = 0; k < 16; k++) {
            u64 s = wsum[k];
            if (k < w) wb += s;
            tot += s;
        }
        u64 carry = carry_s;
        if (i < n_tiles) tile_sums[i] = carry + wb + inc - v;
        __syncthreads();
        if (threadIdx.x == 0) carry_s = carry + tot;
        __syncthreads();
    }
    if (threadIdx.x == 0) *total = carry_s;
}

template <typename F, typename G>
__global__ __launch_bounds__(256) void scan_apply_kernel(F f, G g, u64 n, const u64 *tile_sums, const u32 *np) {
    __shared__ u64 sm[4];
    if (np) {
        const u64 d = *np;
        n = d < n ? d : n;
    }
    if ((u64)blockIdx.x * SCAN_TILE >= n) return;
    u64 base = (u64)blockIdx.x * SCAN_TILE;
    u64 run = tile_sums[blockIdx.x];
#pragma unroll
    for (int k = 0; k < 8; k++) {
        u64 i = base + (u64)k * 256 + threadIdx.x;
        u64 v = i < n ? f(i) : 0;
        u64 tot;
        u64 ex = block_escan_256<u64>(v, sm, &tot);
        if (i < n) g(i, v, run + ex);
        run += tot;
    }
}

constexpr u32 SCAN2_MAX_TILES = 4096;
template <typename F, typename G>
__global__ __launch_bounds__(256) void scan_apply2_kernel(F f, G g, u64 n, const u64 *tile_sums, const u32 *np, u64 *total) {
    __shared__ u64 sm[4];
    __shared__ u64 s_pref[4];
    if (np) {
        const u64 d = *np;
        n = d < n ? d : n;
    }
    const u64 n_tiles = n == 0 ? 1 : (n + SCAN_TILE - 1) / SCAN_TILE;
    if (blockIdx.x >= n_tiles) return;
    u64 acc = 0;
    for (u32 t = threadIdx.x; t < blockIdx.x; t += 256) acc += tile_sums[t];
    acc = wave_sum(acc);
    if (lane_id() == 0) s_pref[threadIdx.x >> 6] = acc;
    __syncthreads();
    u64 run = s_pref[0] + s_pref[1] + s_pref[2] + s_pref[3];
    if (blockIdx.x == n_tiles - 1 && threadIdx.x == 0) *total = run + tile_sums[blockIdx.x];
    const u64 base = (u64)blockIdx.x * SCAN_TILE;
#pragma unroll
    for (int k = 0; k < 8; k++) {
        u64 i = base + (u64)k * 256 + threadIdx.x;
        u64 v = i < n ? f(i) : 0;
// ... 118 lines not shown
```

### portcullis_amd/csrc/pjb_host.hip.h

```cpp
#pragma once
#include "pjb_device.hip.h"
#include "pjb_extra_types.hip.h"

#include <algorithm>
#include <sys/mman.h>
#include <thread>
#include <chrono>
#include <cstdarg>
#include <cstdio>
#include <cstdlib>
#include <cstring>
#include <map>
#include <memory>
#include <mutex>
#include <string>
#include <thread>
#include <vector>

using namespace pjb;


inline thread_local std::string g_create_error;
inline thread_local std::string g_thread_error;
inline thread_local const void *g_thread_error_ctx = nullptr;
// ... 103 lines not shown
    bool run_sort = false;
};

struct CtlSlot {
    Buf cstats, err, gencount, batches, rows;
    Buf x_q, x_spos, x_send, x_gapoff, x_zlist, x_scnt, x_codes;
    Buf tile_cnt, tile_stats, splidx, splpoff, splrec, tile_soff, chunk_tile;
    Buf scan_parts;
    u32 scan_epoch = 0;
    Buf members;
    Buf okey, rec, g, jidbam;
    hipEvent_t ev_k1 = nullptr;
    hipEvent_t ev_xk1 = nullptr;
    Buf total, bitmap, wrank, ends, firstid, key[2], idx[2], hist, hist_scan, hist_part, bintotal, scan_tiles;
    Buf runs;
    Buf pagecnt, pagerank;
    Buf jid, seg, runfirst, runstart, ent, entsum, frag, fragj, acc, ancl, ancr, jkey, genlist, masks;
    bool dense_at_rest = false;
    hipStream_t main = nullptr, side = nullptr;
    hipEvent_t ev_fork = nullptr, ev_join = nullptr, ev_fork2 = nullptr, ev_join2 = nullptr;
    uint8_t *pub = nullptr, *pub_dev = nullptr;
    DevBatch *batches_pinned = nullptr;
    size_t batches_pinned_cap = 0;
    bool at_rest = false;
    hipEvent_t ev[PJB_N_STAGES + 2] = {};
    hipEvent_t ev_rows = nullptr, ev_done = nullptr;
};
struct EvPool {
    std::vector<hipEvent_t> ev;
    size_t used = 0;
    std::vector<int> name;
};
constexpr int MISC_POOL = PJB_MAX_QUEUED;

struct Flight {
    int32_t tid = -1;
    std::vector<int32_t> tids;
    std::vector<int32_t> voff;
    int64_t vlen = 0;
    std::vector<u32> tile_lo;
    std::vector<int64_t> m_reads;
    std::vector<DevBatch> batches;
    std::vector<int> batch_member;
    int slot = 0;
    bool queued = false;
    bool empty = false;
    bool forked = false;
    ContigLimits lim;
    int64_t n_reads = 0;
    u32 n_tiles = 0;
    int attempt = 0, list_attempt = 0;
    int n_pass = 0;
    const u32 *sidx = nullptr;
    const u32 *jid_sorted = nullptr;
    Pairs pr;
    bool x_pre = false;
    bool x_k1 = false;
    int32_t *x_spos = nullptr, *x_send = nullptr;
    u32 *x_gapoff = nullptr;
    Gap *x_gaps = nullptr;
    u32 x_gap_cap = 0;
};

inline void release(Buf &b) {
    if (b.p) (void)hipFree(b.p);
    b.p = nullptr;
    b.cap = 0;
}

struct ModelState {
    Buf g_rows, g_models, g_refs, g_out, g_bad;
    Buf r_nodes, r_leaf, r_roots, r_data, r_pred, r_colmap;
    int32_t r_trees = 0, r_classes = 0, r_vars = 0, r_dep = 0;
    Buf w_pool, w_pack;
    u32 grow_batch = 0;
    Buf n_data, n_part_d, n_part_i, n_out;
    u32 knn_chunk = 0;
    struct GrowOut {
        std::vector<uint8_t> is_ordered;
        std::vector<int64_t> tree_off, count_off;
        std::vector<int32_t> left, right, split_var;
        std::vector<double> split_value, counts, class_values;
    } grow_out;
    void release_all() {
        for (Buf *b : {&g_rows, &g_models, &g_refs, &g_out, &g_bad, &r_nodes, &r_leaf, &r_roots, &r_data, &r_pred, &r_colmap, &w_pool, &w_pack,
                       &n_data, &n_part_d, &n_part_i, &n_out})
            release(*b);
    }
};

constexpr size_t PJB_UP_EVENTS = 64;
struct pjb_ctx {
    pjb_config cfg;
    hipStream_t stream = nullptr;
    hipStream_t stream3 = nullptr;
    hipStream_t stream4 = nullptr;
    hipEvent_t ev_front = nullptr;
    CtlSlot sl[PJB_MAX_QUEUED];
    bool slot_busy[PJB_MAX_QUEUED] = {};
    Flight fl[PJB_MAX_QUEUED];
    int n_fl = 0;
    int cur_slot = 0;
    EvPool pools[PJB_MAX_QUEUED + 1];
    int cur_pool = MISC_POOL;
    Buf b_cursor;
    std::map<int32_t, struct BamStage *> bam_stage;
    std::mutex bam_mu, err_mu;
    std::vector<Buf> genome_pool;
    std::vector<Buf> stage_pool;
    std::vector<Buf> out_pool, misc_pool;
    hipStream_t inf_streams[4] = {};
    unsigned inf_next = 0;
    hipStream_t stream_up = nullptr;
    hipEvent_t ev_up = nullptr;
    hipEvent_t up_events[64] = {};
    int64_t up_ticket = 0, up_done = 0;
    std::string err;
    std::vector<int32_t> ref_len;
    std::vector<Contig> contigs;
    int32_t cur_tid = -1;
    std::map<int32_t, OpenContig> open;
    std::vector<Slab> slab_pool;
    uint8_t *stage[2] = {nullptr, nullptr};
    size_t stage_cap[2] = {0, 0};
    hipEvent_t stage_ev[2] = {nullptr, nullptr};
    bool stage_busy[2] = {false, false};
    unsigned stage_next = 0;
    pjb_junction_row *rows_pinned = nullptr;
    pjb_junction_row *rows_table = nullptr;
    bool rows_copy_pending = false;
    int last_slot = 0;
    int inflate_lanes = 512 * 64;
    bool side_stream = true;
    bool dense_ids = true;
    u32 junc_seen = 0;
    int lbits_seen = 18;
    size_t rows_n = 0, rows_cap = 0;
    size_t rows_pinned_cap = 0;
    std::vector<void *> graveyard;
    std::mutex grave_mu;
    size_t last_rows_n = 0;
    uint8_t *mirror = nullptr;
    size_t mirror_cap = 0;
    int64_t *mirror_hdr = nullptr;
    size_t mirror_rows = 0;
    int64_t mirror_acc[5] = {0, 0, 0, INT32_MAX, 0};
    pjb_timing timing;
    int radix_max_bits = 11;
    double junc_per_read = 0;
    u32 sort_floor = 1u << 16;
    bool window_skip = true;
    bool run_sort = true;
    u32 run_window = 0;
    u32 list_cap_forced = 0;
    bool k1_serial = true;
    hipEvent_t last_k1_ev = nullptr;
    int k1s_blocks_forced = 0;
    bool ktime = false;
    std::vector<std::string> knames;
    std::vector<int64_t> kcount;
    std::vector<double> kms;
    std::vector<std::string> ktime_only;
    Buf *scan_tiles = nullptr;
    Buf b_scan_tiles;
    Buf b_inf_comp, b_inf_out, b_inf_blocks, b_inf_status, b_inf_scratch, b_inf_bitmap;
    Buf b_dfl_in, b_dfl_sym, b_dfl_slots, b_dfl_size, b_dfl_off, b_dfl_packed;
    Buf b_bam_seg, b_bam_rec, b_bam_ctl;
    struct IndexState *index = nullptr;
    bool extra = false;
    std::vector<ExtraContig> xc;
    std::map<int32_t, std::pair<u64 *, u32>> filter_keys;
    Buf f_pos, f_cigoff, f_cigar, f_codes;
    ModelState model;
    Buf x_pos, x_endx, x_q, x_prefq, x_ce, x_bound, x_de, x_dropped, x_zlist, x_cnt, x_tabk, x_tabc, x_rs, x_re, x_rr, x_tileoff;
    Buf x_xrall, x_tab;
    size_t x_tab_slots = 0, x_tab_n = 0;
    XArena xarena;
    pjb_extra_row *xrows_pinned = nullptr;
    size_t xrows_pinned_cap = 0;
    bool extra_dense_only = false;
    Buf b_hasx, b_xtotal;
    Buf b_fasta_raw;
};


inline int fail(pjb_ctx *c, int code, const char *fmt, ...) {
    char tmp[1024];
    va_list ap;
    va_start(ap, fmt);
    vsnprintf(tmp, sizeof tmp, fmt, ap);
    va_end(ap);
    if (c) {
        g_thread_error = tmp;
        g_thread_error_ctx = c;
        std::lock_guard<std::mutex> lk(c->err_mu);
        c->err = tmp;
    } else
        g_create_error = tmp;
    return code;
}

#define HIP_TRY(c, call)                                                                                   \
    do {                                                                                                   \
        hipError_t e_ = (call);                                                                            \
        if (e_ != hipSuccess)                                                                              \
            return fail((c), PJB_ERR_HIP, "%s failed: %s (%s:%d)", #call, hipGetErrorString(e_), __FILE__, \
                        __LINE__);                                                                         \
    } while (0)

inline void bury(pjb_ctx *c, void *p) {
    std::lock_guard<std::mutex> lk(c->grave_mu);
    c->graveyard.push_back(p);
}
inline bool exhume(pjb_ctx *c) {
    std::vector<void *> g;
    {
        std::lock_guard<std::mutex> lk(c->grave_mu);
        g.swap(c->graveyard);
    }
    for (void *p : g) (void)hipFree(p);
    return !g.empty();
}
#ifdef PJB_DEBUG_ALLOC
#define ensure(c, b, bytes) ensure_named((c), (b), (bytes), #b, __LINE__)
inline int ensure_named(pjb_ctx *c, Buf &b, size_t bytes, const char *what, int line);
inline int ensure_impl(pjb_ctx *c, Buf &b, size_t bytes);
inline int ensure_named(pjb_ctx *c, Buf &b, size_t bytes, const char *what, int line) {
    const void *was = b.p;
    const int rc = ensure_impl(c, b, bytes);
    if (b.p != was) fprintf(stderr, "[alloc] %s (line %d): %p .. %p (%zu bytes, asked %zu)\n", what, line, b.p, (void *)((char *)b.p + b.cap), b.cap, bytes);
    return rc;
}
inline int ensure_impl(pjb_ctx *c, Buf &b, size_t bytes) {
#else
inline int ensure(pjb_ctx *c, Buf &b, size_t bytes) {
#endif
    if (bytes <= b.cap && b.p) return PJB_OK;
    if (b.p) bury(c, b.p);
    b.p = nullptr;
    b.cap = 0;
    size_t want = std::max<size_t>(bytes + bytes / 4, 256);
    hipError_t e = hipMalloc(&b.p, want);
    if (e != hipSuccess) {
        (void)hipGetLastError();
        if (exhume(c)) e = hipMalloc(&b.p, want);
    }
    if (e != hipSuccess) {
        want = std::max<size_t>(bytes, 256);
        e = hipMalloc(&b.p, want);
        if (e != hipSuccess) return fail(c, PJB_ERR_NOMEM, "hipMalloc(%zu) failed: %s", want, hipGetErrorString(e));
    }
    b.cap = want;
    static const bool poison = getenv("PJB_POISON") != nullptr && strcmp(getenv("PJB_POISON"), "0") != 0;
    if (poison) {
        (void)hipMemset(b.p, 0xCD, want);
        (void)hipDeviceSynchronize();
    }
    return PJB_OK;
}

inline const char *err_text(int code) {
    switch (code) {
    case PJB_ERR_BAD_XS: return "Unknown strand: XS tag is not one of + - ? .";
    case PJB_ERR_NO_PRESENCE: return "Found an alignment that does not have a presence in the requested region";
    case PJB_ERR_ZERO_LEN_OP: return "Can't extract cigar op sequence from query string when length has been calculated as 0";
    case PJB_ERR_QUERY_RANGE: return "Can't extract cigar op sequence from query string";
    case PJB_ERR_GENOME_RANGE: return "Can't extract cigar op sequence from extracted genome region";
    case PJB_ERR_QREGION: return "Query region is outside the genomic region";
    case PJB_ERR_ANCHOR_MISMATCH: return "Anchor region for query and genome are not the same size";
    case PJB_ERR_SPLICE_SITE_LEN: return "Retrieved sequence for splice site of junction is not the expected length";
    case PJB_ERR_ANCHOR_LEN: return "Retrieved sequence for anchor of junction is not the expected length";
    case PJB_ERR_INTRON_FLANK_LEN: return "Retrieved sequence for intron region of junction is not the expected length";
    case PJB_ERR_MIN_ANCHOR: return "The intron must lie inside its anchors (Intron::minAnchorLength)";
    case PJB_ERR_HAMMING_LEN: return "Can't find hamming distance of strings that are not the same length";
    case PJB_ERR_CLIP_RANGE: return "Soft clip longer than the read (basic_string::substr)";
    case PJB_ERR_UNSORTED: return "Alignments are not coordinate sorted";
    case PJB_ERR_DIVERGENT: return "Malformed CIGAR: padded query and genome walks disagree";
    case PJB_ERR_NO_SEQ: return "A spliced alignment was submitted without its sequence";
    default: return "unknown error";
    }
}

inline int check_device_error(pjb_ctx *c, u64 e) {
    if (e == ~0ull) return PJB_OK;
    const int code = -(int)(e & 0xff);
    const unsigned long long ord = e >> 8;
    return fail(c, code, "%s (alignment ordinal %llu on target %d)", err_text(code), ord, c->cur_tid);
}

inline double wall_now() { return std::chrono::duration<double>(std::chrono::steady_clock::now().time_since_epoch()).count(); }

inline void parallel_copy(void *dst, const void *src, size_t bytes) {
    const size_t MIN_SLICE = (size_t)4 << 20;
    const unsigned hw = std::max(1u, std::thread::hardware_concurrency());
    const size_t nthr = std::min<size_t>(std::min<size_t>(8, hw), bytes / MIN_SLICE);
    if (nthr <= 1) {
        memcpy(dst, src, bytes);
        return;
    }
    std::vector<std::thread> th;
    const size_t per = ((bytes + nthr - 1) / nthr + 63) & ~(size_t)63;
    for (size_t t = 0; t < nthr; t++) {
        const size_t a = std::min(bytes, per * t), b = std::min(bytes, a + per);
        if (a < b) th.emplace_back([=] { memcpy((uint8_t *)dst + a, (const uint8_t *)src + a, b - a); });
    }
    for (auto &x : th) x.join();
// ... 197 lines not shown
```

### portcullis_amd/csrc/pjb_kernels.hip.h

```cpp
#pragma once

#include "pjb_device.hip.h"

namespace pjb {

__global__ __launch_bounds__(256) void k0_upper(uint8_t *g, int64_t n, int do_upper, int *has_x) {
    int64_t i = ((int64_t)blockIdx.x * 256 + threadIdx.x) * 16;
    bool x = false;
    for (int64_t j = i; j < n && j < i + 16; j++) {
        uint8_t c = g[j];
        x |= (c == 'X' || (do_upper && c == 'x'));
    }
    if (__ballot(x) && lane_id() == 0) atomicOr(has_x, 1);
    if (!do_upper) return;
    if (i + 16 <= n && ((uintptr_t)(g + i) & 15) == 0) {
        uint4 v = *reinterpret_cast<uint4 *>(g + i);
        u32 *w = reinterpret_cast<u32 *>(&v);
#pragma unroll
        for (int k = 0; k < 4; k++) {
            u32 x = w[k], r = 0;
#pragma unroll
            for (int b = 0; b < 4; b++) {
                u32 c = (x >> (8 * b)) & 0xff;
                if (c >= 'a' && c <= 'z') c -= 32;
// ... 1744 lines not shown
        ctx.cand_flush(item0 + gridDim.x * K1E_T >= n_items);
    }
}

__global__ __launch_bounds__(256) void kg_member_stats(const u32 *tile_off, const TileStats *ts, const u32 *tile_lo, int n_members, MemberStats *out, u32 n_tiles,
                                                       const ContigStats *cs) {
    __shared__ u64 sm[4][4];
    __shared__ int32_t smi[4][2];
    const int m = blockIdx.x;
    if (m >= n_members) return;
    u64 spl = 0, uns = 0, sum = 0, pairs = 0;
    int32_t mn = INT32_MAX, mx = 0;
    for (u32 t = tile_lo[m] + threadIdx.x; t < tile_lo[m + 1]; t += 256) {
        const TileStats x = ts[t];
        spl += x.spliced;
        uns += x.unspliced;
        sum += x.sum_len;
        mn = min(mn, x.min_len);
        mx = max(mx, x.max_len);
    }
    spl = wave_sum(spl);
    uns = wave_sum(uns);
    sum = wave_sum(sum);
    {
        const u32 t0 = tile_lo[m], t1 = tile_lo[m + 1], total = (u32)cs->n_pairs;
        pairs = threadIdx.x == 0 ? (u64)((t1 < n_tiles ? tile_off[t1] : total) - (t0 < n_tiles ? tile_off[t0] : total)) : 0ull;
    }
    mn = wave_min(mn);
    mx = wave_max(mx);
    const int w = threadIdx.x >> 6;
    if (lane_id() == 0) {
        sm[w][0] = spl;
        sm[w][1] = uns;
        sm[w][2] = sum;
        sm[w][3] = pairs;
        smi[w][0] = mn;
        smi[w][1] = mx;
    }
    __syncthreads();
    if (threadIdx.x == 0) {
        MemberStats S;
        S.spliced = sm[0][0] + sm[1][0] + sm[2][0] + sm[3][0];
        S.unspliced = sm[0][1] + sm[1][1] + sm[2][1] + sm[3][1];
        S.sum_len = sm[0][2] + sm[1][2] + sm[2][2] + sm[3][2];
        S.n_pairs = sm[0][3] + sm[1][3] + sm[2][3] + sm[3][3];
        S.min_len = min(min(smi[0][0], smi[1][0]), min(smi[2][0], smi[3][0]));
        S.max_len = max(max(smi[0][1], smi[1][1]), max(smi[2][1], smi[3][1]));
        S.n_junc = 0;
        S._pad = 0;
        out[m] = S;
    }
}

constexpr int DENSE_ENDS = 8;
constexpr u32 DENSE_EMPTY = 0xffffffffu;

__device__ __forceinline__ u32 start_rank(const u64 *bitmap, const u32 *wrank, int32_t start) {
    const u32 w = (u32)start >> 6;
    return wrank[w] + (u32)__popcll(bitmap[w] & ((1ull << (start & 63)) - 1ull));
}
struct PopcFn {
    const u64 *words;
    __device__ u64 operator()(u64 i) const { return (u64)__popcll(words[i]); }
};
__global__ __launch_bounds__(256) void kd_ends(const u64 *cand, KeyFmt kf, const u64 *bitmap, const u32 *wrank, u32 junc_limit, u32 *ends,
                                               u32 *cand_rank, ContigStats *cs) {
    const u32 n = cs->n_cand;
    for (u32 p = blockIdx.x * 256 + threadIdx.x; p < n; p += gridDim.x * 256) {
        int32_t s, e;
        unpack_key(kf, cand[p], s, e);
        const u32 rs = start_rank(bitmap, wrank, s);
        cand_rank[p] = rs;
        if (rs >= junc_limit) {
            atomicOr(&cs->overflow, OVF_JUNC);
            continue;
        }
        u32 *slot = ends + (size_t)rs * DENSE_ENDS;
        const u32 ue = (u32)e;
        bool placed = false;
        for (int k = 0; k < DENSE_ENDS && !placed; k++) {
            const u32 cur = atomicCAS(&slot[k], DENSE_EMPTY, ue);
            placed = cur == DENSE_EMPTY || cur == ue;
        }
        if (!placed) atomicOr(&cs->overflow, OVF_DENSE);
    }
}
__global__ __launch_bounds__(256) void kd_rank_pages(const u64 *bitmap, const u32 *page_cnt, const u32 *page_rank, u32 *wrank, u32 n_pages, u32 n_words) {
    const u32 page = blockIdx.x * 4 + (threadIdx.x >> 6);
    if (page >= n_pages) return;
    if (page_cnt[page] == 0) return;
    const u32 w = (page << KD_PAGE_SHIFT) + (u32)lane_id();
    const u32 c = w < n_words ? (u32)__popcll(bitmap[w]) : 0u;
    const u32 inc = wave_iscan(c);
    if (w < n_words) wrank[w] = page_rank[page] + inc - c;
}
__global__ __launch_bounds__(256) void kd_reset(const u64 *cand, const u32 *cand_rank, KeyFmt kf, u32 junc_limit, const ContigStats *cs,
                                                u64 *bitmap, u32 *ends, u32 *page_cnt) {
    const u32 n = cs->n_cand;
    for (u32 p = blockIdx.x * 256 + threadIdx.x; p < n; p += gridDim.x * 256) {
        int32_t s, e;
        unpack_key(kf, cand[p], s, e);
        bitmap[(u32)s >> 6] = 0;
        page_cnt[(u32)s >> (6 + KD_PAGE_SHIFT)] = 0;
        const u32 rs = cand_rank[p];
        if (rs < junc_limit) {
            uint4 *q = reinterpret_cast<uint4 *>(ends + (size_t)rs * DENSE_ENDS);
            q[0] = q[1] = make_uint4(DENSE_EMPTY, DENSE_EMPTY, DENSE_EMPTY, DENSE_EMPTY);
        }
    }
}
struct EndsCountFn {
    const u32 *ends;
    __device__ u64 operator()(u64 rs) const {
        const uint4 *q = reinterpret_cast<const uint4 *>(ends + rs * DENSE_ENDS);
        const uint4 a = q[0], b = q[1];
        return (u64)((a.x != DENSE_EMPTY) + (a.y != DENSE_EMPTY) + (a.z != DENSE_EMPTY) + (a.w != DENSE_EMPTY) + (b.x != DENSE_EMPTY) +
                     (b.y != DENSE_EMPTY) + (b.z != DENSE_EMPTY) + (b.w != DENSE_EMPTY));
    }
};
struct FirstIdSink {
    u32 *first_id;
    int32_t *anc_l, *anc_r;
    __device__ void operator()(u64 i, u64, u64 ex) const {
        first_id[i] = (u32)ex;
        anc_l[i] = INT32_MAX;
        anc_r[i] = INT32_MIN;
    }
};
__device__ __forceinline__ u32 ends_below(const u32 *ends, u32 rs, u32 ue) {
    const uint4 *q = reinterpret_cast<const uint4 *>(ends + (size_t)rs * DENSE_ENDS);
    const uint4 a = q[0], b = q[1];
    return (a.x < ue) + (a.y < ue) + (a.z < ue) + (a.w < ue) + (b.x < ue) + (b.y < ue) + (b.z < ue) + (b.w < ue);
}
__device__ __forceinline__ void anchors_fold(bool valid, u32 j, int32_t l, int32_t r, int32_t *anc_l, int32_t *anc_r) {
    const u32 lk = (u32)l ^ 0x80000000u, rk = (u32)r ^ 0x80000000u;
    u64 todo = __ballot(valid);
    while (todo) {
        const int first = __ffsll((long long)todo) - 1;
        const u32 jc = (u32)__builtin_amdgcn_readlane((int)j, first);
        const bool mine = valid && j == jc;
        const u64 m = __ballot(mine);
        const int32_t lo = (int32_t)(wave_total<DppMin>(mine ? lk : 0xffffffffu) ^ 0x80000000u);
        const int32_t hi = (int32_t)(wave_total<DppMax>(mine ? rk : 0u) ^ 0x80000000u);
        if (lane_id() == first) {
            if (lo < __hip_atomic_load(&anc_l[jc], __ATOMIC_RELAXED, __HIP_MEMORY_SCOPE_AGENT)) atomicMin(&anc_l[jc], lo);
            if (hi > __hip_atomic_load(&anc_r[jc], __ATOMIC_RELAXED, __HIP_MEMORY_SCOPE_AGENT)) atomicMax(&anc_r[jc], hi);
        }
        todo &= ~m;
    }
}

__global__ __launch_bounds__(256) void kd_table(const u64 *cand, const u64 *cand_anc, const u32 *cand_rank, KeyFmt kf, u32 junc_limit, const u32 *ends,
                                                const u32 *first_id, const u64 *total, u64 *jkey, int32_t *anc_l, int32_t *anc_r, ContigStats *cs,
                                                const u32 *gen_cnt, u32 gen_cap, u32 sort_limit, u32 *n_runs) {
    const u32 p = blockIdx.x * 256 + threadIdx.x;
    if (blockIdx.x == 0) {
        static_assert(GEN_SHARDS == 256, "a shard per thread of the first block");
        const u32 over = lists_over(gen_cnt, threadIdx.x, gen_cap);
        if (over) atomicMax(&cs->list_need, over);
        if (__syncthreads_or((int)over) && threadIdx.x == 0) cs->overflow |= OVF_LISTS;
    }
    if (p == 0) {
        if (n_runs) *n_runs = 0;
        const u64 J = *total;
        u32 ovf = cs->overflow;
        if (cs->P != 0 && (J > (u64)junc_limit || J > (u64)sort_limit)) {
            ovf |= OVF_JUNC;
            cs->overflow = ovf;
            cs->n_junc = (u32)(J < 0xffffffffull ? J : 0xffffffffull);
        }
        if (ovf) cs->P = 0;
        else if (cs->P) {
            const u32 n_pairs = cs->P;
            cs->n_junc = cs->J = (u32)J;
            cs->n_slices = (n_pairs + 63) / 64;
            cs->n_slots = (u32)J + (n_pairs + 63) / 64;
        }
    }
    const u32 n = cs->n_cand;
    for (u32 base = blockIdx.x * 256u; base < n; base += gridDim.x * 256u) {
        const u32 q = base + threadIdx.x;
        const bool on = q < n;
        const u32 pc = on ? q : n - 1;
        const u32 rs = cand_rank[pc];
        const u64 k = cand[pc], a = cand_anc[pc];
        bool valid = on && rs < junc_limit;
        u32 id = 0xffffffffu;
        if (valid) {
            int32_t s, e;
            unpack_key(kf, k, s, e);
            id = first_id[rs] + ends_below(ends, rs, (u32)e);
            valid = id < junc_limit;
            if (valid) jkey[id] = k;
        }
        if (valid) {
            const int32_t lo = (int32_t)(u32)a, hi = (int32_t)(u32)(a >> 32);
            if (lo < __hip_atomic_load(&anc_l[id], __ATOMIC_RELAXED, __HIP_MEMORY_SCOPE_AGENT)) atomicMin(&anc_l[id], lo);
            if (hi > __hip_atomic_load(&anc_r[id], __ATOMIC_RELAXED, __HIP_MEMORY_SCOPE_AGENT)) atomicMax(&anc_r[id], hi);
        }
    }
}

enum {
    F_N = 0, F_R1P, F_R1N, F_R2P, F_R2N, F_MS, F_XSP, F_XSN, F_UM, F_BPP, F_PPP, F_REL, F_DIST,
    F_MAXMINANC, F_UP, F_DOWN, F_MAXMMES, F_MAXMINMATCH,
    F_FIRSTMIS,
    F_PAD19,
    F_MISM_LO, F_MISM_HI,
    F_JAD0,
    F_WORDS = 48
};
__device__ __forceinline__ void acc_rest_state(u32 *acc, u64 n_junc) {
    const u64 n = n_junc * F_WORDS, step = (u64)gridDim.x * blockDim.x;
    for (u64 t = (u64)blockIdx.x * blockDim.x + threadIdx.x; t < n; t += step) acc[t] = (t % F_WORDS) == F_FIRSTMIS ? 100000000u : 0u;
}

constexpr int KDA_TILE = 4096;
__device__ __forceinline__ void wave_hist_add(u32 *h, u32 d, bool valid);
constexpr int KDA_PER = 4;
constexpr u32 RUN_W = 2048;
struct RunOut {
    u64 *key;
    u32 *cnt;
    u32 *tile_first;
    u32 *tile_n;
    u32 *n_runs;
    u32 cap;
    u32 window;
    int tile_bits;
};
static_assert(RUN_W == 256 * 8, "kd_assign compacts eight table entries a thread");
__device__ __forceinline__ void runs_close_chain(ContigStats *cs) {
    atomicOr(&cs->overflow, OVF_RUNS);
    cs->P = 0;
    cs->J = 0;
    cs->n_slots = 0;
    cs->n_slices = 0;
}
__global__ __launch_bounds__(256) void kd_assign(const u64 *key, const u32 *np, KeyFmt kf, const u64 *bitmap, const u32 *wrank, const u32 *ends,
                                                 const u32 *first_id, u32 junc_limit, const u64 *total, u32 *jid_bam, u32 *acc, const u64 *jkey,
                                                 const int32_t *anc_l, const int32_t *anc_r, u64 *err, ContigStats *cs_chk, int hist_bits, u32 *hist,
                                                 RunOut ro) {
    __shared__ u32 s_h[4096];
    __shared__ u32 s_run[4];
    __shared__ u32 s_rscan[4];
    const u32 n = *np;
    if (n == 0) {
        if (hist_bits > 0)
            for (u32 d = threadIdx.x; d < (1u << hist_bits); d += 256) hist[(size_t)blockIdx.x * (1u << hist_bits) + d] = 0;
        return;
    }
    {
        const u64 J = *total;
        acc_rest_state(acc, J < (u64)junc_limit ? J : (u64)junc_limit);
    }
    const u32 nb = hist_bits > 0 ? 1u << hist_bits : 0u;
    for (u32 d = threadIdx.x; d < (ro.window ? RUN_W : nb); d += 256) s_h[d] = 0;
    if (threadIdx.x == 0) {
        s_run[0] = 0xffffffffu;
        s_run[1] = 0u;
    }
    if (nb || ro.window) __syncthreads();
    u32 id_lo = 0xffffffffu, id_hi = 0u;
    for (u32 chunk = blockIdx.x * (KDA_TILE / (KDA_PER * 256)); chunk < (blockIdx.x + 1) * (KDA_TILE / (KDA_PER * 256)); chunk++) {
    if (chunk * (KDA_PER * 256) >= n) break;
    u64 kk[KDA_PER];
    u32 pp[KDA_PER];
#pragma unroll
    for (int q = 0; q < KDA_PER; q++) {
        pp[q] = (chunk * KDA_PER + q) * 256 + threadIdx.x;
        kk[q] = key[pp[q] < n ? pp[q] : n - 1];
    }
    bool lead[KDA_PER];
    int32_t ss[KDA_PER], ee[KDA_PER];
    u64 bw[KDA_PER];
    u32 wr[KDA_PER];
#pragma unroll
    for (int q = 0; q < KDA_PER; q++) {
        const u32 plo = (u32)__builtin_amdgcn_update_dpp(0, (int)(u32)kk[q], 0x138, 0xf, 0xf, false);
        const u32 phi = (u32)__builtin_amdgcn_update_dpp(0, (int)(u32)(kk[q] >> 32), 0x138, 0xf, 0xf, false);
        lead[q] = lane_id() == 0 || plo != (u32)kk[q] || phi != (u32)(kk[q] >> 32);
        unpack_key(kf, kk[q], ss[q], ee[q]);
        bw[q] = 0;
        wr[q] = 0;
        if (lead[q]) {
            bw[q] = bitmap[(u32)ss[q] >> 6];
            wr[q] = wrank[(u32)ss[q] >> 6];
        }
    }
    u32 rs_[KDA_PER], fi[KDA_PER], eb[KDA_PER];
#pragma unroll
    for (int q = 0; q < KDA_PER; q++) {
        rs_[q] = wr[q] + (u32)__popcll(bw[q] & ((1ull << (ss[q] & 63)) - 1ull));
        fi[q] = eb[q] = 0;
        if (lead[q]) {
            fi[q] = first_id[rs_[q]];
            eb[q] = ends_below(ends, rs_[q], (u32)ee[q]);
        }
    }
#pragma unroll
    for (int q = 0; q < KDA_PER; q++) {
        const u64 lm = __ballot(lead[q]) & ((2ull << lane_id()) - 1ull);
        const u32 id = (u32)__shfl((int)(fi[q] + eb[q]), 63 - __clzll((long long)lm), 64);
        fi[q] = id;
        eb[q] = 0;
        if (pp[q] < n) jid_bam[pp[q]] = id;
        if (nb) wave_hist_add(s_h, id & (nb - 1u), pp[q] < n);
        if (ro.window) {
            wave_hist_add(s_h, id & (RUN_W - 1u), pp[q] < n);
            if (pp[q] < n) {
                id_lo = id < id_lo ? id : id_lo;
                id_hi = id > id_hi ? id : id_hi;
            }
        }
    }
#ifdef PJB_SELFCHECK
    const u32 p = pp[0];
    if (p < n) {
    const int32_t s = ss[0], e = ee[0];
    const u32 rs = rs_[0], id = fi[0] + eb[0];
    {
        int bad = 0;
        const uint4 *q = reinterpret_cast<const uint4 *>(ends + (size_t)rs * DENSE_ENDS);
        const uint4 a = q[0], b = q[1];
        const u32 ue = (u32)e;
        if (!((bitmap[(u32)s >> 6] >> (s & 63)) & 1ull)) bad = 6;
        else if (!(a.x == ue || a.y == ue || a.z == ue || a.w == ue || b.x == ue || b.y == ue || b.z == ue || b.w == ue)) bad = 7;
        else if (id >= junc_limit || id >= (u32)*total) bad = 1;
        else if (jkey[id] != key[p]) bad = 2;
// ... 243 lines not shown
        if (d < nb) {
            mine += (u32)wcnt[d] + wcnt[nb + d] + wcnt[2 * nb + d] + wcnt[3 * nb + d];
            below += k < RS_PF ? pf_rt[k < RS_PF ? k : 0] : row_total[d];
        }
    }
    u64 tot;
    const u64 both = block_escan_256<u64>((u64)mine | ((u64)below << 32), s_scan, &tot);
    u32 tstart = (u32)both, dbase = (u32)(both >> 32);
    for (u32 k = 0; k < per; k++) {
        const u32 d = d0 + k;
        if (d >= nb) break;
        const u32 c0 = wcnt[d], c1 = wcnt[nb + d], c2 = wcnt[2 * nb + d], c3 = wcnt[3 * nb + d];
        const u32 gfirst = dbase + (k < RS_PF ? pf_hs[k < RS_PF ? k : 0] : hist_scan[(size_t)tile * nb + d]);
        dbase += k < RS_PF ? pf_rt[k < RS_PF ? k : 0] : row_total[d];
        delta[d] = gfirst - tstart;
        wcnt[d] = (unsigned short)tstart;
        wcnt[nb + d] = (unsigned short)(tstart + c0);
        wcnt[2 * nb + d] = (unsigned short)(tstart + c0 + c1);
        wcnt[3 * nb + d] = (unsigned short)(tstart + c0 + c1 + c2);
        tstart += c0 + c1 + c2 + c3;
    }
    __syncthreads();
#pragma unroll
    for (int r = 0; r < RS_ITEMS; r++) {
        const u32 i = base + r * 64 + lane;
        const u32 lp = ((rkp[r >> 1] >> ((r & 1) * 16)) & 0xffffu) + wc[(u32)(key[r] >> shift) & mask];
        rkp[r >> 1] = (r & 1) ? ((rkp[r >> 1] & 0xffffu) | (lp << 16)) : ((rkp[r >> 1] & 0xffff0000u) | lp);
        if (i < n) kbuf[lp] = key[r];
    }
    __syncthreads();
    const u32 cnt = min((u32)RS_TILE, n - tile * RS_TILE);
    u32 digp[RS_ITEMS / 2];
#pragma unroll
    for (int r = 0; r < RS_ITEMS; r++) {
        const u32 j = r * 256 + threadIdx.x;
        const K kk = j < cnt ? kbuf[j] : (K)0;
        const u32 d = (u32)(kk >> shift) & mask;
        digp[r >> 1] = (r & 1) ? (digp[r >> 1] | (d << 16)) : d;
        if (j < cnt) kout[delta[d] + j] = kk;
    }
    __syncthreads();
#pragma unroll
    for (int r = 0; r < RS_ITEMS; r++) {
        const u32 i = base + r * 64 + lane;
        if (i < n) ibuf[(rkp[r >> 1] >> ((r & 1) * 16)) & 0xffffu] = val[r];
    }
    __syncthreads();
#pragma unroll
    for (int r = 0; r < RS_ITEMS; r++) {
        const u32 j = r * 256 + threadIdx.x;
        if (j < cnt) vout[delta[(digp[r >> 1] >> ((r & 1) * 16)) & 0xffffu] + j] = ibuf[j];
    }
}

struct RunCountFn {
    const u32 *cnt, *order;
    __device__ u64 operator()(u64 i) const { return cnt[order[i]]; }
};
struct RunDestSink {
    u32 *dest;
    const u32 *order;
    __device__ void operator()(u64 i, u64, u64 ex) const { dest[order[i]] = (u32)ex; }
};
__global__ __launch_bounds__(256) void rs_place(const u32 *jid_bam, const u32 *np, const u64 *run_key, const u32 *run_dest, const u32 *tile_first,
                                                const u32 *tile_n, u32 run_cap, int tile_bits, u32 *kout, u32 *vout) {
    __shared__ u32 s_dest[RUN_W];
    __shared__ unsigned short s_wcnt[4][RUN_W];
    const u32 n = *np;
    const u32 tile = blockIdx.x;
    if ((u64)tile * RS_TILE >= n) return;
    for (u32 d = threadIdx.x; d < 2 * RUN_W; d += 256) ((u32 *)&s_wcnt[0][0])[d] = 0;
    const u32 tf = tile_first[tile], tn = tf < run_cap ? min(tile_n[tile], min(RUN_W, run_cap - tf)) : 0u;
    for (u32 e = threadIdx.x; e < tn; e += 256) s_dest[(u32)(run_key[tf + e] >> tile_bits) & (RUN_W - 1u)] = run_dest[tf + e];
    const int w = __builtin_amdgcn_readfirstlane(threadIdx.x >> 6), lane = lane_id();
    unsigned short *wc = s_wcnt[w];
    const u32 base = tile * RS_TILE + w * (RS_TILE / 4);
    const u64 lt = (1ull << lane) - 1;
    u32 id[RS_ITEMS];
    u32 rkp[RS_ITEMS / 2];
    const u32 *kp = jid_bam + base;
#pragma unroll
    for (int r = 0; r < RS_ITEMS; r++) id[r] = kp[r * 64 + lane];
    __syncthreads();
#pragma unroll
    for (int r = 0; r < RS_ITEMS; r++) {
        const bool valid = base + r * 64 + lane < n;
        const u32 d = id[r] & (RUN_W - 1u);
        u32 rank = 0;
        u64 todo = __ballot(valid);
        while (todo) {
            const int first = __ffsll((long long)todo) - 1;
            const u32 idc = (u32)__builtin_amdgcn_readlane((int)id[r], first);
            const bool mine = valid && id[r] == idc;
            const u64 m = __ballot(mine);
            u32 before = 0;
            if (lane == first) {
                before = wc[d];
                wc[d] = (unsigned short)(before + (u32)__popcll(m));
            }
            before = (u32)__builtin_amdgcn_readlane((int)before, first);
            if (mine) rank = before + (u32)__popcll(m & lt);
            todo &= ~m;
        }
        rkp[r >> 1] = (r & 1) ? (rkp[r >> 1] | (rank << 16)) : rank;
    }
    __syncthreads();
#pragma unroll
    for (int r = 0; r < RS_ITEMS; r++) {
        const u32 i = base + r * 64 + lane;
        const u32 d = id[r] & (RUN_W - 1u);
        u32 dst = s_dest[d] + ((rkp[r >> 1] >> ((r & 1) * 16)) & 0xffffu);
        for (int q = 0; q < w; q++) dst += s_wcnt[q][d];
        if (i < n && dst < n) {
            kout[dst] = id[r];
            vout[dst] = i;
        }
    }
}

struct HeadFn {
    const u64 *skey;
    const u32 *sidx;
    const PairRec *rec;
    __device__ u64 operator()(u64 i) const {
        const u64 im = i ? i - 1 : 0;
        const u64 ka = skey[i], kb = skey[im];
        const u32 sa = sidx[i], sb = sidx[im];
        const int32_t pa = rec[sa].pos, pb = rec[sb].pos;
        const bool hj = i == 0 || ka != kb;
        const bool hr = hj || pa != pb;
        return ((u64)hj << 32) | (u64)hr;
    }
};
struct HeadSink {
    u32 *jid_of;
    u32 *seg_off;
    u32 *run_first;
    u32 *run_start;
    const u64 *skey;
    u64 *jkey;
    u32 junc_limit;
    __device__ void operator()(u64 i, u64 v, u64 ex) const {
        const u32 j = (u32)(ex >> 32) + (u32)(v >> 32) - 1;
        const u32 r = (u32)ex + (u32)v - 1;
        jid_of[i] = j;
        if (v >> 32) {
            seg_off[j] = (u32)i;
            run_first[j] = r;
            if (jkey && j < junc_limit) jkey[j] = skey[i];
        }
        if ((u32)v) run_start[r] = (u32)i;
    }
};
__global__ void k2_close(u64 *total, u32 *seg_off, u32 *run_first, u32 *run_start, ContigStats *cs, u32 junc_limit, const u32 *gen_cnt, u32 gen_cap) {
    const u32 n_pairs = cs->P;
    if (n_pairs == 0) return;
    {
        u32 need = 0;
        for (u32 sh = 0; sh < GEN_SHARDS; sh++) need = max(need, lists_over(gen_cnt, sh, gen_cap));
        if (need) {
            cs->list_need = need;
            cs->overflow |= OVF_LISTS;
            cs->P = 0;
            return;
        }
    }
    const u32 J = (u32)(*total >> 32), R = (u32)*total;
    cs->n_junc = J;
    cs->n_runs = R;
    if (J > junc_limit) {
        cs->overflow |= OVF_JUNC;
        cs->P = 0;
        return;
    }
    seg_off[J] = n_pairs;
    run_first[J] = R;
    run_start[R] = n_pairs;
    cs->J = J;
    cs->R = R;
    cs->n_slots = J + (n_pairs + 63) / 64;
}

struct Popc64Fn {
    const u64 *words;
    __device__ u64 operator()(u64 i) const { return (u64)__popcll(words[i]); }
};
constexpr int K2E_PER = 4;
__global__ __launch_bounds__(256) void k2_expand(const u32 *sid, const u64 *head_mask, const u64 *run_mask, const u32 *run_base, const u64 *total,
                                                 u32 *seg_off, u32 *run_first, u32 *run_start, ContigStats *cs) {
    const u32 n = cs->P;
#pragma unroll
    for (int q = 0; q < K2E_PER; q++) {
        const u32 i = (blockIdx.x * K2E_PER + q) * 256 + threadIdx.x;
        if (i >= n) continue;
        const u32 sl = i >> 6, bit = i & 63u;
        const u64 mr = run_mask[sl], mj = head_mask[sl];
        if ((mr >> bit) & 1ull) {
            const u32 r = run_base[sl] + (u32)__popcll(mr & ((1ull << bit) - 1ull));
            run_start[r] = i;
            if ((mj >> bit) & 1ull) {
                const u32 j = sid[i];
                seg_off[j] = i;
                run_first[j] = r;
            }
        }
    }
    if (n > 0 && (n - 1) / (256u * K2E_PER) == blockIdx.x && threadIdx.x == 0) {
        const u32 R = (u32)*total, J = cs->J;
        seg_off[J] = n;
        run_first[J] = R;
        run_start[R] = n;
        cs->n_runs = cs->R = R;
    }
}

__global__ __launch_bounds__(256) void kf_init(u32 *acc, const u32 *n_junc_p, int32_t *anc_l, int32_t *anc_r) {
    const u32 n_junc = *n_junc_p;
    acc_rest_state(acc, n_junc);
    for (u64 t = (u64)blockIdx.x * 256 + threadIdx.x; t < n_junc; t += (u64)gridDim.x * 256) {
        anc_l[t] = INT32_MAX;
        anc_r[t] = INT32_MIN;
    }
}
__global__ __launch_bounds__(256) void kf_anchors(const u32 *sidx, const u32 *jid_of, const PairRec *rec, const u32 *np, u32 *jid_bam, int32_t *anc_l,
                                                   int32_t *anc_r) {
    const u32 n = *np;
    if (blockIdx.x * 256u >= n) return;
    const u32 i = blockIdx.x * 256 + threadIdx.x;
    const bool valid = i < n;
    const u32 ic = valid ? i : n - 1;
    const u32 p = sidx[ic], j = jid_of[ic];
    const uint4 ra = *reinterpret_cast<const uint4 *>(rec + p);
    if (valid) jid_bam[p] = j;
    anchors_fold(valid, j, (int32_t)ra.z, (int32_t)ra.w, anc_l, anc_r);
}

constexpr int GENERIC_NW = 8;
struct Side {
    int32_t len, mism, first_mis, last_mis;
    int err;
};

__device__ Side anchor_side(const OpsView cig, u32 n, int32_t position, int32_t aligned, const uint8_t *seq, int32_t lq,
                            const uint8_t *genome, int32_t glen, bool genome_has_x, const u32 *gcodes, int32_t start,
                            int32_t end, u32 k0, int32_t r0, int32_t q0, int32_t q_limit ) {
    Side S;
    S.len = 0;
    S.mism = 0;
    S.first_mis = -1;
    S.last_mis = -1;
    S.err = 0;
    const int32_t get_end = position + aligned - 1;
    if (start > get_end || end < position) {
        S.err = PJB_ERR_NO_PRESENCE;
        return S;
    }
    int32_t dS = 0, dE = 0;
    if ((cig[0] & 15u) == OP_S) dS = (int32_t)(cig[0] >> 4);
    if ((cig[n - 1] & 15u) == OP_S) dE = (int32_t)(cig[n - 1] >> 4);
    if (dS > lq) {
        S.err = PJB_ERR_CLIP_RANGE;
        return S;
    }
    const u64 cnt = (u64)(int64_t)lq - (u64)(int64_t)dS - (u64)(int64_t)dE + 1ull;
    const u64 avail = (u64)(lq - dS);
    const int32_t clen = (int32_t)(cnt < avail ? cnt : avail);
    int32_t rPos = r0, qPos = q0;
    for (u32 k = k0; k < n; k++) {
        const u32 op = cig[k], ty = op & 15u;
        const int32_t ln = (int32_t)(op >> 4);
        const bool cRef = op_consumes_ref(ty);
        const bool cQry = op_consumes_query(ty) && ty != OP_S;
        if (rPos < start) {
            if (cRef) rPos += ln;
            if (cQry) qPos += ln;
            continue;
        }
        if ((rPos > end && ty != OP_I) || (ty == OP_N && rPos + ln > end)) break;
        if (cQry) {
            const int32_t l = (rPos + ln > end && ty != OP_I) ? end - rPos + 1 : ln;
            if (l == 0) {
                S.err = PJB_ERR_ZERO_LEN_OP;
                return S;
            }
            if (qPos < 0 || qPos + l > clen) {
                S.err = PJB_ERR_QUERY_RANGE;
                return S;
            }
        }
        if (cRef) rPos += ln;
        if (cQry) qPos += ln;
    }
    const int32_t q_start = position > start ? position : start;
    const int32_t q_end = rPos <= end ? rPos - 1 : end;
    if (q_start - start < 0 || end - q_end < 0) {
        S.err = PJB_ERR_QREGION;
        return S;
    }
    const int32_t gsize = end - start + 1;
    rPos = r0;
    qPos = q0;
    bool qDone = false, gDone = false, diverged = false;
    int32_t qTot = 0, gTot = 0, mism = 0, first_mis = -1, last_mis = -1;
    for (u32 k = k0; k < n; k++) {
        const u32 op = cig[k], ty = op & 15u;
        const int32_t ln = (int32_t)(op >> 4);
        const bool cRef = op_consumes_ref(ty);
        const bool cQry = op_consumes_query(ty) && ty != OP_S;
        int32_t qEmit = 0, gEmit = 0;
        int qKind = 0, gKind = 0;
        if (!qDone && rPos >= start) {
            if ((rPos > end && ty != OP_I) || (ty == OP_N && rPos + ln > end)) qDone = true;
            else if (cQry) {
                qEmit = (rPos + ln > end && ty != OP_I) ? end - rPos + 1 : ln;
                qKind = 1;
            } else if (cRef) {
                qEmit = rPos + ln > end ? end - rPos + 1 : ln;
                qKind = 2;
            }
        }
        if (!gDone && rPos >= q_start) {
            if (rPos > q_end && ty != OP_I) gDone = true;
            else if (cRef) {
                const int32_t so = rPos - start;
                gEmit = rPos + ln > q_end ? q_end - rPos + 1 : ln;
                if (so < 0 || so + gEmit > gsize) {
                    S.err = PJB_ERR_GENOME_RANGE;
                    return S;
                }
                gKind = 1;
            } else if (cQry) {
                gEmit = ln;
                gKind = 2;
// ... 53 lines not shown
        return S;
    }
    S.len = qTot;
    S.mism = mism;
    S.first_mis = first_mis;
    S.last_mis = last_mis;
    return S;
}

__device__ __forceinline__ u64 pair_stats_generic(const OpsView cig, u32 nc, int32_t pos, int32_t aligned, const uint8_t *seq,
                                                  int32_t lq, const uint8_t *genome, int32_t glen, bool has_x, const u32 *gcodes,
                                                  int32_t left, int32_t istart, int32_t iend, int32_t right, u32 g, u64 *err, u32 opi,
                                                  int32_t qN, int32_t q_limit) {
    if (lq <= 1) {
        const u32 totUp = (u32)((istart - 1) - left + 1);
        const u32 totDown = (u32)(right - (iend + 1) + 1);
        return pack_res(0, totUp < totDown ? totUp : totDown, 0);
    }
    u32 kL = opi, kR = 0;
    int32_t rL = istart, qL = qN, rR = pos, qR = 0;
    while (kL > 0) {
        const u32 op = cig[kL - 1], ty = op & 15u;
        const int32_t ln = (int32_t)(op >> 4);
        const int32_t rp = rL - (op_consumes_ref(ty) ? ln : 0);
        if (rp < left) break;
        kL--;
        rL = rp;
        if (op_consumes_query(ty) && ty != OP_S) qL -= ln;
    }
    const int32_t after = istart + (int32_t)(cig[opi] >> 4);
    if (after == iend + 1) {
        kR = opi + 1;
        rR = after;
        qR = qN;
    }
    const Side L = anchor_side(cig, nc, pos, aligned, seq, lq, genome, glen, has_x, gcodes, left, istart - 1, kL, rL, qL, q_limit);
    if (L.err) {
        set_error(err, g, L.err);
        return 0;
    }
    const Side R = anchor_side(cig, nc, pos, aligned, seq, lq, genome, glen, has_x, gcodes, iend + 1, right, kR, rR, qR, q_limit);
    if (R.err) {
        set_error(err, g, R.err);
        return 0;
    }
    const u32 upM = L.last_mis < 0 ? (u32)L.len : (u32)(L.len - 1 - L.last_mis);
    const u32 downM = R.first_mis < 0 ? (u32)R.len : (u32)R.first_mis;
    const u32 tu = (u32)(L.len - L.mism), td = (u32)(R.len - R.mism);
    return pack_res(upM < downM ? upM : downM, tu < td ? tu : td, (u32)(L.mism + R.mism));
}

__global__ __launch_bounds__(256) void k4b_generic(const u64 *list, const u32 *gen_cnt, u32 cap, const u64 *key, PairRec *rec, const u32 *jid_bam,
                                                    KeyFmt kf, const DevBatch *batches, int n_batches, const int32_t *anc_l, const int32_t *anc_r,
                                                    GroupTab G, int genome_has_x, int use_codes, u64 *err, const ContigStats *cs, u32 pack_nn,
                                                    const u32 *spl_idx, const uint4 *spl_rec) {
    __shared__ u32 s_ops[OPS_LDS][256];
    __shared__ u32 s_first[2 * GEN_SHARDS + 1];
    __shared__ u32 s_wsum[4];
    __shared__ BatchTab s_bt;
    if (cs->P == 0) return;
    {
        const u32 i0 = threadIdx.x * 2;
        const u32 c0 = gen_cnt[(i0 % GEN_SHARDS) * GEN_CNT_STRIDE + (i0 / GEN_SHARDS) * 2];
        const u32 c1 = gen_cnt[((i0 + 1) % GEN_SHARDS) * GEN_CNT_STRIDE + ((i0 + 1) / GEN_SHARDS) * 2];
        const u32 n0 = c0 < cap ? c0 : cap, n1 = c1 < cap ? c1 : cap;
        s_bt.fill(batches, n_batches);
        u32 total;
        const u32 ex = block_escan<4>(n0 + n1, s_wsum, &total);
        s_first[i0] = ex;
        s_first[i0 + 1] = ex + n0;
        if (threadIdx.x == 255) s_first[2 * GEN_SHARDS] = total;
        __syncthreads();
    }
    static_assert(GEN_SHARDS == 256, "two sub-lists per thread of the block");
    const u32 n_items = s_first[2 * GEN_SHARDS];
    for (u32 item0 = blockIdx.x * 256; item0 < n_items; item0 += gridDim.x * 256) {
    const u32 item = item0 + threadIdx.x;
    if (item >= n_items) continue;
    u32 sub = 0;
#pragma unroll
    for (u32 step = GEN_SHARDS; step > 0; step >>= 1)
        if (sub + step < 2 * GEN_SHARDS && s_first[sub + step] <= item) sub += step;
    const bool check_only = sub >= GEN_SHARDS;
    const u64 entry = list[(size_t)sub * cap + (item - s_first[sub])];
    const u32 p0 = (u32)(entry >> 32);
    const u32 slot = check_only && pack_nn ? (u32)entry & 0x0fffffffu : (u32)entry;
    if (check_only) {
        const u32 code = pack_nn ? (u32)entry >> 28 : 15u;
        const u32 nN = code < 15u ? code : (reinterpret_cast<const uint4 *>(rec + p0)[1].w >> 16) + 1u;
        bool ok = true;
        int32_t prev_istart = 0, is, ie;
        unpack_key(kf, key[p0], is, ie);
        for (u32 k = 0; k < nN; k++) {
            const u32 j = jid_bam[p0 + k];
            int32_t nis = 0, nie = 0;
            if (k + 1 < nN) unpack_key(kf, key[p0 + k + 1], nis, nie);
            if (k > 0 && prev_istart >= anc_l[j]) ok = false;
            if (k + 1 < nN && nie + 1 <= anc_r[j]) ok = false;
            prev_istart = is;
            is = nis;
            ie = nie;
        }
        if (ok) continue;
    }
    const int bi = s_bt.find(batches, n_batches, slot / (u32)K1_TILE);
    const DevBatch &b = batches[bi];
    const u32 r = spl_idx[slot];
    const uint4 sr = spl_rec[slot];
    const u32 g = gload(&b.base) + r;
    const u32 c0 = sr.x;
    u32 nc = sr.w & 0x7fffu;
    if (nc == 0x7fffu) nc = gload(b.cig_off + r + 1) - c0;
    OpsView cig;
    cig.g = b.cigar + c0;
    cig.lds = &s_ops[0][threadIdx.x];
    {
        u32 w[OPS_LDS];
        fetch_ops8(as_global(b.cigar), c0, s_bt.cig_words(b, bi), w);
#pragma unroll
        for (int k = 0; k < OPS_LDS; k++) s_ops[k][threadIdx.x] = (u32)k < nc ? w[k] : 0u;
    }
    const uint4 rb = reinterpret_cast<const uint4 *>(rec + p0)[1];
    const int32_t vpos = (int32_t)rb.x, aend = (int32_t)rb.y;
    const Member M = member_of(G, vpos);
    const int32_t pos = vpos - M.voff;
    int32_t lq = (int32_t)(sr.w >> 16);
    if (lq == 0xffff) lq = gload(b.l_qseq + r);
    const u32 so0 = sr.z;
    if (lq > 1 && !(sr.w & 0x8000u)) {
        set_error(err, g, PJB_ERR_NO_SEQ);
        continue;
    }
    const uint8_t *seq = b.seq4 + (size_t)so0 * 4;
    const int32_t q_limit = (int32_t)min(s_bt.seq_words(b, bi) - 1u - so0, 0x7fffffffu);
    u32 k = 0;
    int32_t qsum = 0;
    for (u32 i = 0; i < nc; i++) {
        const u32 op = cig[i], ty = op & 15u;
        if (ty == OP_N) {
            const u32 p = p0 + k;
            const u32 j = jid_bam[p];
            int32_t istart, iend;
            unpack_key(kf, key[p], istart, iend);
            const u64 res = pair_stats_generic(cig, nc, pos, aend - vpos + 1, seq, lq, M.d, M.len, genome_has_x != 0, use_codes ? M.codes : (const u32 *)nullptr,
                                               anc_l[j] - M.voff, istart - M.voff, iend - M.voff, anc_r[j] - M.voff, g, err, i, qsum, q_limit);
            *reinterpret_cast<u64 *>(rec + p) = res;
            k++;
        }
        if (op_consumes_query(ty) && ty != OP_S) qsum += (int32_t)(op >> 4);
    }
    }
}

__global__ __launch_bounds__(256) void k4_pairs(const u32 *sidx, const u32 *jid_of, const PairRec *rec, const u64 *jkey, KeyFmt kf, const u32 *np,
                                                 u32 *frag, int32_t *frag_j, u64 *head_mask, u64 *run_mask, const ContigStats *cs_chk, u64 *err_chk) {
    const u32 n = *np;
    if (blockIdx.x * 256u >= n) return;
    const u32 i = blockIdx.x * 256 + threadIdx.x;
    const bool valid = i < n;
    const int lane = lane_id();
    const u32 ic = valid ? i : n - 1;
    const u32 p = sidx[ic];
    const u32 jv = jid_of[ic];
#ifdef PJB_SELFCHECK
    {
        const u32 Jc = cs_chk->J;
        const u32 jb = ic ? jid_of[ic - 1] : jv;
        int bad = 0;
        if (p >= n) bad = 1;
        else if (jv >= Jc) bad = 2;
        else if (jv != jb && jv != jb + 1) bad = 3;
        else if (ic == 0 && jv != 0) bad = 4;
        else if (ic == n - 1 && jv != Jc - 1) bad = 5;
        else if (jv + (ic >> 6) + 1 >= cs_chk->n_slots) bad = 6;
        else if ((ic >> 6) >= cs_chk->n_slices) bad = 7;
        else if (cs_chk->n_slots != Jc + (n + 63) / 64) bad = 8;
        if (__ballot(bad != 0)) {
            if (bad) set_error(err_chk, 0xffffe000u + (u32)bad, PJB_ERR_HIP);
            return;
        }
    }
#endif
    const PairRec Rc = rec_load(rec + p);
    const u64 jk = jkey[jv];
    u32 jprev_v = __shfl_up(jv, 1, 64);
    int32_t pos_prev = __shfl_up(Rc.pos, 1, 64), aend_prev = __shfl_up(Rc.aend, 1, 64);
    if (lane == 0 && valid && i > 0) {
        jprev_v = jid_of[i - 1];
        const uint4 q = reinterpret_cast<const uint4 *>(rec + sidx[i - 1])[1];
        pos_prev = (int32_t)q.x;
        aend_prev = (int32_t)q.y;
    }
    u32 j = 0xffffffffu;
    u32 cnt[4] = {0, 0, 0, 0}, jadp[5] = {0, 0, 0, 0, 0}, mx[5] = {0, 0, 0, 0, 0};
    u32 first_mis = 100000000u;
    u64 mism64 = 0;
    if (valid) {
        j = jv;
        int32_t istart, iend;
        unpack_key(kf, jk, istart, iend);
        const u64 rs = Rc.aux;
        const u32 minMatch = (u32)(rs & 0xfffffu), mmes = (u32)((rs >> 20) & 0xfffffu), nbMis = (u32)(rs >> 40);
        const u32 meta = Rc.meta;
        const u32 cat = meta & META_CAT_MASK;
        const u32 xs = (meta >> META_XS_SHIFT) & 3u;
        const bool dist_head = i == 0 || jprev_v != j || pos_prev != Rc.pos || aend_prev != Rc.aend;
        cnt[0] = 1u | ((u32)(cat == 0) << 8) | ((u32)(cat == 1) << 16) | ((u32)(cat == 2) << 24);
        cnt[1] = (u32)(cat == 3) | ((u32)((meta & META_MULTI) != 0) << 8) | ((u32)(xs == 1) << 16) | ((u32)(xs == 2) << 24);
        cnt[2] = (u32)((meta & META_UM) != 0) | ((u32)((meta & META_BPP) != 0) << 8) | ((u32)((meta & META_PPP) != 0) << 16) |
                 ((u32)((meta & META_REL) != 0) << 24);
        cnt[3] = (u32)dist_head;
#pragma unroll
        for (int w = 0; w < 5; w++)
            jadp[w] = (u32)((u32)(4 * w) < minMatch) | ((u32)((u32)(4 * w + 1) < minMatch) << 8) |
                      ((u32)((u32)(4 * w + 2) < minMatch) << 16) | ((u32)((u32)(4 * w + 3) < minMatch) << 24);
        const int32_t la = istart - Rc.lstart, ra = Rc.rend - iend;
        mx[0] = (u32)(la < ra ? la : ra);
        mx[1] = Rc.updown & 0xffffu;
        mx[2] = Rc.updown >> 16;
        mx[3] = mmes;
        mx[4] = minMatch;
        first_mis = minMatch > 0 ? minMatch : 100000000u;
        mism64 = nbMis;
        if (lane == 0 && i > 0 && jprev_v != j) frag_j[j + (i >> 6) - 1] = -1;
        if (i == n - 1) frag_j[j + (i >> 6) + 1] = -1;
    }
    if (head_mask) {
        const bool hj = valid && (i == 0 || jprev_v != j);
        const bool hr = valid && (hj || pos_prev != Rc.pos);
        const u64 mj = __ballot(hj), mr = __ballot(hr);
        if (lane == 0 && i < n) {
            head_mask[i >> 6] = mj;
            run_mask[i >> 6] = mr;
        }
    }
    auto store_fragment = [&](u32 hi_word) {
        const u32 slot = j + (i >> 6);
        u32 vals[F_WORDS];
#pragma unroll
        for (int k = 0; k < F_WORDS; k++) vals[k] = 0;
#pragma unroll
        for (int k = 0; k < 13; k++) vals[F_N + k] = (cnt[k >> 2] >> (8 * (k & 3))) & 0xffu;
        vals[F_MAXMINANC] = mx[0];
        vals[F_UP] = mx[1];
        vals[F_DOWN] = mx[2];
        vals[F_MAXMMES] = mx[3];
        vals[F_MAXMINMATCH] = mx[4];
        vals[F_FIRSTMIS] = first_mis;
        vals[F_MISM_LO] = (u32)mism64;
        vals[F_MISM_HI] = hi_word;
#pragma unroll
        for (int k = 0; k < 20; k++) vals[F_JAD0 + k] = (jadp[k >> 2] >> (8 * (k & 3))) & 0xffu;
        uint4 *dst = reinterpret_cast<uint4 *>(frag + (size_t)slot * F_WORDS);
#pragma unroll
        for (int k = 0; k < F_WORDS / 4; k++) dst[k] = make_uint4(vals[4 * k], vals[4 * k + 1], vals[4 * k + 2], vals[4 * k + 3]);
        frag_j[slot] = (int32_t)j;
    };
    const u32 j0 = (u32)__builtin_amdgcn_readfirstlane((int)j);
    if (__ballot(valid && j != j0) == 0) {
#pragma unroll
        for (int w = 0; w < 4; w++) cnt[w] = wave_total<DppAdd>(cnt[w]);
#pragma unroll
        for (int w = 0; w < 5; w++) jadp[w] = wave_total<DppAdd>(jadp[w]);
#pragma unroll
        for (int w = 0; w < 5; w++) mx[w] = wave_total<DppMax>(mx[w]);
        first_mis = wave_total<DppMin>(first_mis);
        mism64 = (u64)wave_total<DppAdd>((u32)mism64);
        if (valid && lane == 0) store_fragment(0u);
        return;
    }
    u32 take = 0;
#pragma unroll
    for (int sft = 0; sft < 6; sft++) {
        const int o = 1 << sft;
        const u32 kk = __shfl_down(j, o, 64);
        if (lane + o < 64 && kk == j) take |= 1u << sft;
    }
    auto red_add = [&](u32 v) {
#pragma unroll
        for (int sft = 0; sft < 6; sft++) {
            const u32 t = __shfl_down(v, 1 << sft, 64);
            if ((take >> sft) & 1u) v += t;
        }
        return v;
    };
    auto red_max = [&](u32 v) {
#pragma unroll
        for (int sft = 0; sft < 6; sft++) {
            const u32 t = __shfl_down(v, 1 << sft, 64);
            if (((take >> sft) & 1u) && t > v) v = t;
        }
        return v;
    };
#pragma unroll
    for (int w = 0; w < 4; w++) cnt[w] = red_add(cnt[w]);
#pragma unroll
    for (int w = 0; w < 5; w++) jadp[w] = red_add(jadp[w]);
#pragma unroll
    for (int w = 0; w < 5; w++) mx[w] = red_max(mx[w]);
#pragma unroll
    for (int sft = 0; sft < 6; sft++) {
        const u32 t = __shfl_down(first_mis, 1 << sft, 64);
        const u64 t64 = __shfl_down(mism64, 1 << sft, 64);
        if ((take >> sft) & 1u) {
            first_mis = t < first_mis ? t : first_mis;
            mism64 += t64;
        }
    }
    const u32 jprev = __shfl_up(j, 1, 64);
    if (valid && (lane == 0 || jprev != j)) store_fragment((u32)(mism64 >> 32));
}

__device__ __forceinline__ u32 frag_combine(int k, u32 a, u32 b) {
    if (k >= F_MAXMINANC && k <= F_MAXMINMATCH) return a > b ? a : b;
    if (k == F_FIRSTMIS) return a < b ? a : b;
    return a + b;
}
constexpr int FRAG_SLOTS_PER_WAVE = 16;
__global__ __launch_bounds__(256) void k5_frag_reduce(const u32 *frag, const int32_t *frag_j, const u32 *n_slots_p, u32 *acc) {
    const u32 n_slots = *n_slots_p;
    const u32 wave = (blockIdx.x * 256 + threadIdx.x) >> 6;
    const int k = lane_id();
    const u32 s0 = wave * FRAG_SLOTS_PER_WAVE;
    if (s0 >= n_slots) return;
    const int32_t myj = (k < FRAG_SLOTS_PER_WAVE && s0 + k < n_slots) ? frag_j[s0 + k] : -1;
    int32_t cur = -1;
    u32 v = 0, carry_lo = 0;
    auto flush = [&](int32_t j) {
        if (j < 0 || k >= F_JAD0 + 20) return;
        u32 *dst = acc + (size_t)j * F_WORDS + k;
        if (k == F_MISM_LO) return;
        if (k == F_MISM_HI) {
            atomicAdd(reinterpret_cast<u64 *>(dst - 1), ((u64)v << 32) | carry_lo);
        } else if (k >= F_MAXMINANC && k <= F_MAXMINMATCH) atomicMax(dst, v);
        else if (k == F_FIRSTMIS) atomicMin(dst, v);
        else if (v) atomicAdd(dst, v);
    };
    u32 row[FRAG_SLOTS_PER_WAVE];
#pragma unroll
    for (int q = 0; q < FRAG_SLOTS_PER_WAVE; q++) {
        const int32_t jq = __shfl(myj, q, 64);
        row[q] = (jq >= 0 && k < F_WORDS) ? frag[(size_t)(s0 + (u32)q) * F_WORDS + k] : 0u;
    }
#pragma unroll
    for (int q = 0; q < FRAG_SLOTS_PER_WAVE; q++) {
        const int32_t j = __shfl(myj, q, 64);
        if (j >= 0) {
            const u32 w = row[q];
            const u32 wlo = __shfl(w, F_MISM_LO, 64);
            if (j != cur) {
                flush(cur);
                cur = j;
                v = w;
                carry_lo = wlo;
            } else if (k == F_MISM_HI) {
                const u64 sum = (((u64)v << 32) | carry_lo) + (((u64)w << 32) | wlo);
                v = (u32)(sum >> 32);
                carry_lo = (u32)sum;
            } else {
                v = frag_combine(k, v, w);
            }
        }
    }
    flush(cur);
}


__global__ __launch_bounds__(256) void k5_entropy_sum(const u32 *seg_off, const u32 *run_first, const u32 *run_start, const u32 *n_junc_p,
                                                       double *ent_sum) {
    const int lane = lane_id(), sl = lane & 15;
    const u32 j = ((blockIdx.x * 4 + (threadIdx.x >> 6)) << 2) + (u32)(lane >> 4);
    const bool valid = j < *n_junc_p;
    const u32 rf = valid ? run_first[j] : 0u, rl = valid ? run_first[j + 1] : 0u;
    const u32 n = valid ? seg_off[j + 1] - seg_off[j] : 0u;
    double sum = 0.0;
    for (u32 r0 = rf; __any(r0 < rl); r0 += 16) {
        const u32 r = r0 + (u32)sl;
        double t = 0.0;
        if (r < rl) {
            u32 c = run_start[r + 1] - run_start[r];
            if (rl - rf > 1) {
                if (r == rf) c += 1;
                else if (r == rl - 1) c -= 1;
            }
            if (c != 0 && n > 1) {
                const double pI = (double)c / (double)n;
                t = __dmul_rn(pI, log2(pI));
            }
        }
        const u32 cnt = r0 < rl ? (rl - r0 < 16u ? rl - r0 : 16u) : 0u;
#pragma unroll
        for (u32 k = 0; k < 16; k++) {
            const double v = __shfl(t, (int)k, 16);
            if (k < cnt) sum = __dadd_rn(sum, v);
        }
    }
    if (valid && sl == 0) ent_sum[j] = sum;
}

__global__ __launch_bounds__(256) void k5_finalize(const u64 *jkey, const u32 *seg_off, const u32 *run_first,
                                                    const u32 *run_start, const u32 *acc, const int32_t *anc_l,
                                                    const int32_t *anc_r, KeyFmt kf, GroupTab G, const u32 *n_junc_p, const double *ent_sum,
                                                    pjb_junction_row *rows, u64 *err, u32 *member_junc) {
    const u32 n_junc = *n_junc_p;
    const u32 j = blockIdx.x * 256 + threadIdx.x;
    if (j >= n_junc) return;
    const u32 *a = acc + (size_t)j * F_WORDS;
    pjb_junction_row R;
    memset(&R, 0, sizeof R);
    int32_t istart, iend;
    unpack_key(kf, jkey[j], istart, iend);
    const Member M = member_of(G, istart);
    const uint8_t *genome = M.d;
    const int32_t glen = M.len;
    istart -= M.voff;
    iend -= M.voff;
    if (G.n > 1) {
        const int m0 = __builtin_amdgcn_readfirstlane(M.idx);
        const u64 same = __ballot(M.idx == m0);
        if (M.idx == m0) {
            if (lane_id() == __ffsll((long long)same) - 1) atomicAdd(&member_junc[m0], (u32)__popcll(same));
        } else
            atomicAdd(&member_junc[M.idx], 1u);
    }
    R.refid = M.tid;
    R.start = istart;
    R.end = iend;
    R.left = anc_l[j] - M.voff;
    R.right = anc_r[j] - M.voff;
    const u32 n = a[F_N];
    R.nb_raw = n;
    R.nb_dist = a[F_DIST];
    R.nb_ms = a[F_MS];
    R.nb_um = a[F_UM];
    R.nb_bpp = a[F_BPP];
    R.nb_ppp = a[F_PPP];
    R.nb_rel = a[F_REL];
    R.r1pos = a[F_R1P];
    R.r1neg = a[F_R1N];
    R.r2pos = a[F_R2P];
    R.r2neg = a[F_R2N];
    R.max_min_anc = a[F_MAXMINANC];
    R.maxmmes = a[F_MAXMMES];
    R.nb_up_juncs = a[F_UP];
    R.nb_down_juncs = a[F_DOWN];
    const u64 mism = (u64)a[F_MISM_LO] | ((u64)a[F_MISM_HI] << 32);
    R.sum_mismatches = mism;
    for (int k = 0; k < 20; k++) R.jad[k] = a[F_JAD0 + k];
    {
        const u32 first_mis = a[F_FIRSTMIS];
        if ((u32)mism > 0 && first_mis < 20 && !(a[F_MAXMINMATCH] > first_mis)) R.suspicious = 1;
    }
    {
        const u32 np = a[F_XSP], nn = a[F_XSN];
        const double tot = (double)n;
        if ((double)np / tot >= 0.95) R.read_strand = PJB_STRAND_POS;
        else if ((double)nn / tot >= 0.95) R.read_strand = PJB_STRAND_NEG;
        else R.read_strand = PJB_STRAND_UNK;
    }
    R.entropy = n > 1 ? fabs(ent_sum[j]) : 0.0;
    {
        int32_t b = istart, e = istart + 1;
        fetch_clamp(glen, b, e);
        int32_t b2 = iend - 1, e2 = iend;
        fetch_clamp(glen, b2, e2);
        if (e - b + 1 != 2 || e2 - b2 + 1 != 2 || glen <= 0) {
            set_error(err, 0xffffff00u + 0, PJB_ERR_SPLICE_SITE_LEN);
            rows[j] = R;
            return;
        }
// ... 161 lines not shown
```

Measured before the change: 30.15 billion reads/s.

## Have each k4_pairs wave walk a range of slices and merge fragments per range

k4_pairs now assigns a range of 2^shift 64-pair slices (default 8) to each wave instead of one slice. The wave loops over the slices with software-prefetched loads, reduces each junction segment with DPP folds through LDS, and carries open fragments across slices. A fragment is emitted per junction per range instead of per slice, which shrinks the fragment table and the k5_frag_reduce atomic work. The slot-count formulas change to match, and the range size can be set by an option or environment variable. The cost is a serial per-segment loop inside each wave and fewer waves in flight for k4.

```diff
diff --git a/portcullis_amd/csrc/pjb_api.hip b/portcullis_amd/csrc/pjb_api.hip
--- a/portcullis_amd/csrc/pjb_api.hip
+++ b/portcullis_amd/csrc/pjb_api.hip
@@ -150,6 +150,11 @@
         int v = atoi(s);
         if (v >= 4 && v <= RS_MAX_BITS) c->radix_max_bits = v;
     }
+    if (const char *s = getenv("PJB_PAIR_RANGE")) {
+        const int v = atoi(s);
+        for (int k = 0; k <= PAIR_RANGE_SHIFT_MAX; k++)
+            if (v == 1 << k) c->pair_range_shift = k;
+    }
     cmark("options");
     attr_thread.join();
     cmark("kernel attributes");
@@ -691,6 +696,12 @@
     else if (n == "run_window") {
         if (value < 0 || value > (int64_t)RUN_W) return fail(c, PJB_ERR_ARG, "set_option: run_window takes 0 (the default, %u) to %u", RUN_W, RUN_W);
         c->run_window = (u32)value;
+    } else if (n == "pair_range") {
+        int shift = -1;
+        for (int k = 0; k <= PAIR_RANGE_SHIFT_MAX; k++)
+            if (value == (int64_t)1 << k) shift = k;
+        if (shift < 0) return fail(c, PJB_ERR_ARG, "set_option: pair_range takes 1, 2, 4, 8, 16 or 32 slices a range (the default: %d)", 1 << PAIR_RANGE_SHIFT_DEFAULT);
+        c->pair_range_shift = shift;
     } else if (n == "grow_batch") {
         if (value < 0 || value > 32768) return fail(c, PJB_ERR_ARG, "set_option: grow_batch takes 0 (the default: what the pool holds) to 32768 trees");
         c->model.grow_batch = (u32)value;
diff --git a/portcullis_amd/csrc/pjb_chain.hip.h b/portcullis_amd/csrc/pjb_chain.hip.h
--- a/portcullis_amd/csrc/pjb_chain.hip.h
+++ b/portcullis_amd/csrc/pjb_chain.hip.h
@@ -46,7 +46,8 @@
     int32_t ref_len;
     KeyFmt kf;
     u32 PL, JL, SL;
-    u32 n_tiles, pair_blocks, slots_lim, n_slices_lim, gen_cap, pack_nn;
+    u32 n_tiles, pair_blocks, range_blocks, slots_lim, n_slices_lim, gen_cap, pack_nn;
+    int range_shift;
     size_t n_words;
     int64_t row_base, mirror_base;
     u32 rs_tiles, run_cap, ro_tiles, plan_tiles;
@@ -133,7 +134,9 @@
     ch.pair_blocks = std::max<u32>(1, (PL + 255) / 256);
     ch.gen_cap = lim.list_cap ? lim.list_cap : (c->list_cap_forced ? c->list_cap_forced : gen_list_cap(PL));
     ch.pack_nn = (u64)ch.n_tiles * K1_TILE < (1ull << 28) ? 1u : 0u;
-    ch.slots_lim = JL + (PL + 63) / 64 + 1;
+    ch.range_shift = c->pair_range_shift;
+    ch.slots_lim = frag_slots_limit(JL, PL, ch.range_shift);
+    ch.range_blocks = std::max<u32>(1, (frag_ranges(PL, ch.range_shift) + 3) / 4);
     ch.n_slices_lim = (PL + 63) / 64 + 1;
     ch.n_words = ((size_t)std::max(ch.ref_len, 1) + 63) / 64;
     ch.stage_events = c->ktime && c->ktime_only.empty();
@@ -438,7 +441,7 @@
         return rc;
     LAUNCH(c, "kd_table", kd_table, dim3(cand_blocks), dim3(256), (const u64 *)cand, (const u64 *)S.ent.p, (const u32 *)cand_rank, kf, JL,
            (const u32 *)S.ends.p, (const u32 *)S.firstid.p, (const u64 *)S.total.p, (u64 *)S.jkey.p, (int32_t *)S.ancl.p, (int32_t *)S.ancr.p, ch.d_cs,
-           (const u32 *)ch.d_gen_cnt, ch.gen_cap, ch.SL, ch.ro.n_runs);
+           (const u32 *)ch.d_gen_cnt, ch.gen_cap, ch.SL, ch.ro.n_runs, ch.range_shift);
     LAUNCH(c, "kd_assign", kd_assign, dim3(ch.rs_tiles), dim3(256), okey, ch.d_P, kf, (const u64 *)S.bitmap.p, (const u32 *)S.wrank.p,
            (const u32 *)S.ends.p, (const u32 *)S.firstid.p, JL, (const u64 *)S.total.p, (u32 *)S.jidbam.p, (u32 *)S.acc.p, (const u64 *)S.jkey.p,
            (const int32_t *)S.ancl.p, (const int32_t *)S.ancr.p, ch.d_err, ch.d_cs, ch.run_route ? 0 : ch.pass_bits[0], (u32 *)S.hist.p, ch.ro);
@@ -579,8 +582,8 @@
 #ifdef PJB_DEBUG_LAUNCH
     debug_sort_check(ch);
 #endif
-    LAUNCH(c, "k4_pairs", k4_pairs, dim3(pair_blocks), dim3(256), f.sidx, f.jid_sorted, (const PairRec *)ch.pr.rec, (const u64 *)S.jkey.p, ch.kf, ch.d_P,
-           (u32 *)S.frag.p, (int32_t *)S.fragj.p, head_mask, run_mask, (const ContigStats *)ch.d_cs, ch.d_err);
+    LAUNCH(c, "k4_pairs", k4_pairs, dim3(ch.range_blocks), dim3(256), f.sidx, f.jid_sorted, (const PairRec *)ch.pr.rec, (const u64 *)S.jkey.p, ch.kf, ch.d_P,
+           (u32 *)S.frag.p, (int32_t *)S.fragj.p, head_mask, run_mask, (const ContigStats *)ch.d_cs, ch.d_err, ch.range_shift);
     if ((rc = run_scan(c, "k2_runs", Popc64Fn{(const u64 *)run_mask}, ExclusiveU32Sink{run_base}, (u64)n_slices_lim, (u64 *)S.total.p, &ch.d_cs->n_slices)))
         return rc;
     LAUNCH(c, "k2_expand", k2_expand, dim3((pair_blocks + K2E_PER - 1) / K2E_PER), dim3(256), f.jid_sorted, (const u64 *)head_mask, (const u64 *)run_mask, (const u32 *)run_base,
@@ -600,7 +603,7 @@
     HeadSink hs{(u32 *)S.jid.p, (u32 *)S.seg.p, (u32 *)S.runfirst.p, (u32 *)S.runstart.p, skey, (u64 *)S.jkey.p, JL};
     if ((rc = run_scan(c, "k2_heads", hf, hs, (u64)ch.PL, (u64 *)S.total.p, ch.d_P))) return rc;
     LAUNCH(c, "k2_close", k2_close, dim3(1), dim3(1), (u64 *)S.total.p, (u32 *)S.seg.p, (u32 *)S.runfirst.p,
-           (u32 *)S.runstart.p, ch.d_cs, JL, (const u32 *)ch.d_gen_cnt, ch.gen_cap);
+           (u32 *)S.runstart.p, ch.d_cs, JL, (const u32 *)ch.d_gen_cnt, ch.gen_cap, ch.range_shift);
     STAGE_EVENT(3);
     if ((rc = chain_fork(ch, S.ev_fork2, S.ev_join2, ch.entropy_forked, chain_entropy))) return rc;
     LAUNCH(c, "kf_init", kf_init, dim3(std::max<u32>(1, std::min<u32>((JL * F_WORDS + 255) / 256, 4096))), dim3(256), (u32 *)S.acc.p, ch.d_J, (int32_t *)S.ancl.p,
@@ -609,8 +612,8 @@
            (int32_t *)S.ancl.p, (int32_t *)S.ancr.p);
     if ((rc = chain_k4b(ch))) return rc;
     STAGE_EVENT(4);
-    LAUNCH(c, "k4_pairs", k4_pairs, dim3(pair_blocks), dim3(256), f.sidx, f.jid_sorted, (const PairRec *)ch.pr.rec, (const u64 *)S.jkey.p, ch.kf, ch.d_P,
-           (u32 *)S.frag.p, (int32_t *)S.fragj.p, (u64 *)nullptr, (u64 *)nullptr, (const ContigStats *)ch.d_cs, ch.d_err);
+    LAUNCH(c, "k4_pairs", k4_pairs, dim3(ch.range_blocks), dim3(256), f.sidx, f.jid_sorted, (const PairRec *)ch.pr.rec, (const u64 *)S.jkey.p, ch.kf, ch.d_P,
+           (u32 *)S.frag.p, (int32_t *)S.fragj.p, (u64 *)nullptr, (u64 *)nullptr, (const ContigStats *)ch.d_cs, ch.d_err, ch.range_shift);
     STAGE_EVENT(5);
     return PJB_OK;
 }
diff --git a/portcullis_amd/csrc/pjb_device.hip.h b/portcullis_amd/csrc/pjb_device.hip.h
--- a/portcullis_amd/csrc/pjb_device.hip.h
+++ b/portcullis_amd/csrc/pjb_device.hip.h
@@ -67,6 +67,24 @@
     u32 max_span;
 };
 static_assert(sizeof(ContigStats) == 112, "ContigStats layout");
+
+constexpr int PAIR_RANGE_SHIFT_MAX = 5;
+constexpr int PAIR_RANGE_SHIFT_DEFAULT = 3;
+__host__ __device__ inline u32 frag_ranges(u32 n_pairs, int range_shift) {
+    return (u32)(((u64)n_pairs + ((u64)64 << range_shift) - 1) >> (6 + range_shift));
+}
+__host__ __device__ inline u32 frag_slot(u32 jid, u32 pair, int range_shift) { return jid + (pair >> (6 + range_shift)); }
+__host__ __device__ inline u32 frag_slots(u32 n_junc, u32 n_pairs, int range_shift) { return n_junc + frag_ranges(n_pairs, range_shift); }
+__host__ __device__ inline int64_t frag_unused_before(u32 jid, u32 pair, bool junction_head, int range_shift) {
+    const bool range_head = (pair & (((u32)64 << range_shift) - 1u)) == 0;
+    return pair != 0 && range_head && junction_head ? (int64_t)frag_slot(jid, pair, range_shift) - 1 : -1;
+}
+__host__ __device__ inline int64_t frag_unused_behind(u32 jid, u32 pair, u32 n_pairs, int range_shift) {
+    return pair + 1 == n_pairs ? (int64_t)frag_slot(jid, pair, range_shift) + 1 : -1;
+}
+__host__ __device__ inline u32 frag_slots_limit(u32 junc_limit, u32 pair_limit, int range_shift) {
+    return frag_slots(junc_limit, pair_limit, range_shift) + 1;
+}
 __device__ __forceinline__ bool window_reach(u32 blk, u32 nl_prev, u32 nl_next, u32 B) {
     const u32 l = __builtin_elementwise_add_sat(blk, nl_prev), r = __builtin_elementwise_add_sat(__builtin_elementwise_add_sat(blk, nl_next), 1u);
     return l <= B || r <= B;
@@ -306,15 +324,17 @@
     __device__ __forceinline__ static u32 op(u32 a, u32 b) { return a < b ? a : b; }
 };
 template <typename Op>
-__device__ __forceinline__ u32 wave_total(u32 v) {
+__device__ __forceinline__ u32 wave_fold(u32 v) {
     v = Op::op(v, dpp_move<0xB1, 0xf>(Op::ident, v));
     v = Op::op(v, dpp_move<0x4E, 0xf>(Op::ident, v));
     v = Op::op(v, dpp_move<0x141, 0xf>(Op::ident, v));
     v = Op::op(v, dpp_move<0x140, 0xf>(Op::ident, v));
     v = Op::op(v, dpp_move<0x142, 0xa>(Op::ident, v));
     v = Op::op(v, dpp_move<0x143, 0xc>(Op::ident, v));
-    return (u32)__builtin_amdgcn_readlane((int)v, 63);
-}
+    return v;
+}
+template <typename Op>
+__device__ __forceinline__ u32 wave_total(u32 v) { return (u32)__builtin_amdgcn_readlane((int)wave_fold<Op>(v), 63); }
 
 template <typename T>
 __device__ __forceinline__ T block_escan_256(T v, T *smem, T *total) {
diff --git a/portcullis_amd/csrc/pjb_host.hip.h b/portcullis_amd/csrc/pjb_host.hip.h
--- a/portcullis_amd/csrc/pjb_host.hip.h
+++ b/portcullis_amd/csrc/pjb_host.hip.h
@@ -279,6 +279,7 @@
     bool window_skip = true;
     bool run_sort = true;
     u32 run_window = 0;
+    int pair_range_shift = PAIR_RANGE_SHIFT_DEFAULT;
     u32 list_cap_forced = 0;
     bool k1_serial = true;
     hipEvent_t last_k1_ev = nullptr;
diff --git a/portcullis_amd/csrc/pjb_kernels.hip.h b/portcullis_amd/csrc/pjb_kernels.hip.h
--- a/portcullis_amd/csrc/pjb_kernels.hip.h
+++ b/portcullis_amd/csrc/pjb_kernels.hip.h
@@ -1920,7 +1920,7 @@
 
 __global__ __launch_bounds__(256) void kd_table(const u64 *cand, const u64 *cand_anc, const u32 *cand_rank, KeyFmt kf, u32 junc_limit, const u32 *ends,
                                                 const u32 *first_id, const u64 *total, u64 *jkey, int32_t *anc_l, int32_t *anc_r, ContigStats *cs,
-                                                const u32 *gen_cnt, u32 gen_cap, u32 sort_limit, u32 *n_runs) {
+                                                const u32 *gen_cnt, u32 gen_cap, u32 sort_limit, u32 *n_runs, int range_shift) {
     const u32 p = blockIdx.x * 256 + threadIdx.x;
     if (blockIdx.x == 0) {
         static_assert(GEN_SHARDS == 256, "a shard per thread of the first block");
@@ -1942,7 +1942,7 @@
             const u32 n_pairs = cs->P;
             cs->n_junc = cs->J = (u32)J;
             cs->n_slices = (n_pairs + 63) / 64;
-            cs->n_slots = (u32)J + (n_pairs + 63) / 64;
+            cs->n_slots = frag_slots((u32)J, n_pairs, range_shift);
         }
     }
     const u32 n = cs->n_cand;
@@ -2492,7 +2492,8 @@
         if ((u32)v) run_start[r] = (u32)i;
     }
 };
-__global__ void k2_close(u64 *total, u32 *seg_off, u32 *run_first, u32 *run_start, ContigStats *cs, u32 junc_limit, const u32 *gen_cnt, u32 gen_cap) {
+__global__ void k2_close(u64 *total, u32 *seg_off, u32 *run_first, u32 *run_start, ContigStats *cs, u32 junc_limit, const u32 *gen_cnt, u32 gen_cap,
+                         int range_shift) {
     const u32 n_pairs = cs->P;
     if (n_pairs == 0) return;
     {
@@ -2518,7 +2519,7 @@
     run_start[R] = n_pairs;
     cs->J = J;
     cs->R = R;
-    cs->n_slots = J + (n_pairs + 63) / 64;
+    cs->n_slots = frag_slots(J, n_pairs, range_shift);
 }
 
 struct Popc64Fn {
@@ -2878,170 +2879,201 @@
     }
 }
 
-__global__ __launch_bounds__(256) void k4_pairs(const u32 *sidx, const u32 *jid_of, const PairRec *rec, const u64 *jkey, KeyFmt kf, const u32 *np,
-                                                 u32 *frag, int32_t *frag_j, u64 *head_mask, u64 *run_mask, const ContigStats *cs_chk, u64 *err_chk) {
-    const u32 n = *np;
-    if (blockIdx.x * 256u >= n) return;
-    const u32 i = blockIdx.x * 256 + threadIdx.x;
-    const bool valid = i < n;
-    const int lane = lane_id();
-    const u32 ic = valid ? i : n - 1;
-    const u32 p = sidx[ic];
-    const u32 jv = jid_of[ic];
-#ifdef PJB_SELFCHECK
-    {
-        const u32 Jc = cs_chk->J;
-        const u32 jb = ic ? jid_of[ic - 1] : jv;
-        int bad = 0;
-        if (p >= n) bad = 1;
-        else if (jv >= Jc) bad = 2;
-        else if (jv != jb && jv != jb + 1) bad = 3;
-        else if (ic == 0 && jv != 0) bad = 4;
-        else if (ic == n - 1 && jv != Jc - 1) bad = 5;
-        else if (jv + (ic >> 6) + 1 >= cs_chk->n_slots) bad = 6;
-        else if ((ic >> 6) >= cs_chk->n_slices) bad = 7;
-        else if (cs_chk->n_slots != Jc + (n + 63) / 64) bad = 8;
-        if (__ballot(bad != 0)) {
-            if (bad) set_error(err_chk, 0xffffe000u + (u32)bad, PJB_ERR_HIP);
-            return;
-        }
-    }
-#endif
-    const PairRec Rc = rec_load(rec + p);
-    const u64 jk = jkey[jv];
-    u32 jprev_v = __shfl_up(jv, 1, 64);
-    int32_t pos_prev = __shfl_up(Rc.pos, 1, 64), aend_prev = __shfl_up(Rc.aend, 1, 64);
-    if (lane == 0 && valid && i > 0) {
-        jprev_v = jid_of[i - 1];
-        const uint4 q = reinterpret_cast<const uint4 *>(rec + sidx[i - 1])[1];
-        pos_prev = (int32_t)q.x;
-        aend_prev = (int32_t)q.y;
-    }
-    u32 j = 0xffffffffu;
-    u32 cnt[4] = {0, 0, 0, 0}, jadp[5] = {0, 0, 0, 0, 0}, mx[5] = {0, 0, 0, 0, 0};
-    u32 first_mis = 100000000u;
-    u64 mism64 = 0;
-    if (valid) {
-        j = jv;
-        int32_t istart, iend;
-        unpack_key(kf, jk, istart, iend);
-        const u64 rs = Rc.aux;
-        const u32 minMatch = (u32)(rs & 0xfffffu), mmes = (u32)((rs >> 20) & 0xfffffu), nbMis = (u32)(rs >> 40);
-        const u32 meta = Rc.meta;
-        const u32 cat = meta & META_CAT_MASK;
-        const u32 xs = (meta >> META_XS_SHIFT) & 3u;
-        const bool dist_head = i == 0 || jprev_v != j || pos_prev != Rc.pos || aend_prev != Rc.aend;
-        cnt[0] = 1u | ((u32)(cat == 0) << 8) | ((u32)(cat == 1) << 16) | ((u32)(cat == 2) << 24);
-        cnt[1] = (u32)(cat == 3) | ((u32)((meta & META_MULTI) != 0) << 8) | ((u32)(xs == 1) << 16) | ((u32)(xs == 2) << 24);
-        cnt[2] = (u32)((meta & META_UM) != 0) | ((u32)((meta & META_BPP) != 0) << 8) | ((u32)((meta & META_PPP) != 0) << 16) |
-                 ((u32)((meta & META_REL) != 0) << 24);
-        cnt[3] = (u32)dist_head;
-#pragma unroll
-        for (int w = 0; w < 5; w++)
-            jadp[w] = (u32)((u32)(4 * w) < minMatch) | ((u32)((u32)(4 * w + 1) < minMatch) << 8) |
-                      ((u32)((u32)(4 * w + 2) < minMatch) << 16) | ((u32)((u32)(4 * w + 3) < minMatch) << 24);
-        const int32_t la = istart - Rc.lstart, ra = Rc.rend - iend;
-        mx[0] = (u32)(la < ra ? la : ra);
-        mx[1] = Rc.updown & 0xffffu;
-        mx[2] = Rc.updown >> 16;
-        mx[3] = mmes;
-        mx[4] = minMatch;
-        first_mis = minMatch > 0 ? minMatch : 100000000u;
-        mism64 = nbMis;
-        if (lane == 0 && i > 0 && jprev_v != j) frag_j[j + (i >> 6) - 1] = -1;
-        if (i == n - 1) frag_j[j + (i >> 6) + 1] = -1;
-    }
-    if (head_mask) {
-        const bool hj = valid && (i == 0 || jprev_v != j);
-        const bool hr = valid && (hj || pos_prev != Rc.pos);
-        const u64 mj = __ballot(hj), mr = __ballot(hr);
-        if (lane == 0 && i < n) {
-            head_mask[i >> 6] = mj;
-            run_mask[i >> 6] = mr;
-        }
-    }
-    auto store_fragment = [&](u32 hi_word) {
-        const u32 slot = j + (i >> 6);
-        u32 vals[F_WORDS];
-#pragma unroll
-        for (int k = 0; k < F_WORDS; k++) vals[k] = 0;
-#pragma unroll
-        for (int k = 0; k < 13; k++) vals[F_N + k] = (cnt[k >> 2] >> (8 * (k & 3))) & 0xffu;
-        vals[F_MAXMINANC] = mx[0];
-        vals[F_UP] = mx[1];
-        vals[F_DOWN] = mx[2];
-        vals[F_MAXMMES] = mx[3];
-        vals[F_MAXMINMATCH] = mx[4];
-        vals[F_FIRSTMIS] = first_mis;
-        vals[F_MISM_LO] = (u32)mism64;
-        vals[F_MISM_HI] = hi_word;
-#pragma unroll
-        for (int k = 0; k < 20; k++) vals[F_JAD0 + k] = (jadp[k >> 2] >> (8 * (k & 3))) & 0xffu;
-        uint4 *dst = reinterpret_cast<uint4 *>(frag + (size_t)slot * F_WORDS);
-#pragma unroll
-        for (int k = 0; k < F_WORDS / 4; k++) dst[k] = make_uint4(vals[4 * k], vals[4 * k + 1], vals[4 * k + 2], vals[4 * k + 3]);
-        frag_j[slot] = (int32_t)j;
-    };
-    const u32 j0 = (u32)__builtin_amdgcn_readfirstlane((int)j);
-    if (__ballot(valid && j != j0) == 0) {
-#pragma unroll
-        for (int w = 0; w < 4; w++) cnt[w] = wave_total<DppAdd>(cnt[w]);
-#pragma unroll
-        for (int w = 0; w < 5; w++) jadp[w] = wave_total<DppAdd>(jadp[w]);
-#pragma unroll
-        for (int w = 0; w < 5; w++) mx[w] = wave_total<DppMax>(mx[w]);
-        first_mis = wave_total<DppMin>(first_mis);
-        mism64 = (u64)wave_total<DppAdd>((u32)mism64);
-        if (valid && lane == 0) store_fragment(0u);
-        return;
-    }
-    u32 take = 0;
-#pragma unroll
-    for (int sft = 0; sft < 6; sft++) {
-        const int o = 1 << sft;
-        const u32 kk = __shfl_down(j, o, 64);
-        if (lane + o < 64 && kk == j) take |= 1u << sft;
-    }
-    auto red_add = [&](u32 v) {
-#pragma unroll
-        for (int sft = 0; sft < 6; sft++) {
-            const u32 t = __shfl_down(v, 1 << sft, 64);
-            if ((take >> sft) & 1u) v += t;
-        }
-        return v;
-    };
-    auto red_max = [&](u32 v) {
-#pragma unroll
-        for (int sft = 0; sft < 6; sft++) {
-            const u32 t = __shfl_down(v, 1 << sft, 64);
-            if (((take >> sft) & 1u) && t > v) v = t;
-        }
-        return v;
-    };
-#pragma unroll
-    for (int w = 0; w < 4; w++) cnt[w] = red_add(cnt[w]);
-#pragma unroll
-    for (int w = 0; w < 5; w++) jadp[w] = red_add(jadp[w]);
-#pragma unroll
-    for (int w = 0; w < 5; w++) mx[w] = red_max(mx[w]);
-#pragma unroll
-    for (int sft = 0; sft < 6; sft++) {
-        const u32 t = __shfl_down(first_mis, 1 << sft, 64);
-        const u64 t64 = __shfl_down(mism64, 1 << sft, 64);
-        if ((take >> sft) & 1u) {
-            first_mis = t < first_mis ? t : first_mis;
-            mism64 += t64;
-        }
-    }
-    const u32 jprev = __shfl_up(j, 1, 64);
-    if (valid && (lane == 0 || jprev != j)) store_fragment((u32)(mism64 >> 32));
-}
-
 __device__ __forceinline__ u32 frag_combine(int k, u32 a, u32 b) {
     if (k >= F_MAXMINANC && k <= F_MAXMINMATCH) return a > b ? a : b;
     if (k == F_FIRSTMIS) return a < b ? a : b;
     return a + b;
 }
+enum { FW_CNT = 0, FW_MAX = 4, FW_MIN = 9, FW_JAD = 10 };
+struct FragWordOf {
+    u32 word, shift, mask;
+    __device__ __forceinline__ explicit FragWordOf(int k) {
+        const bool c = k <= F_DIST, a = k >= F_JAD0 && k < F_JAD0 + 20, m = k >= F_MAXMINANC && k <= F_FIRSTMIS;
+        const int q = a ? k - F_JAD0 : k;
+        word = c ? FW_CNT + (u32)(q >> 2) : a ? FW_JAD + (u32)(q >> 2) : m ? FW_MAX + (u32)(k - F_MAXMINANC) : 15u;
+        shift = c || a ? 8u * (u32)(q & 3) : 0u;
+        mask = c || a ? 0xffu : m ? 0xffffffffu : 0u;
+    }
+    __device__ __forceinline__ static void put(u32 *tot, int quad, bool holder, u32 a, u32 b, u32 c, u32 d) {
+        if (holder) reinterpret_cast<uint4 *>(tot)[quad] = make_uint4(a, b, c, d);
+        __builtin_amdgcn_sched_barrier(0);
+    }
+    __device__ __forceinline__ u32 get(const u32 *tot) const {
+        __builtin_amdgcn_wave_barrier();
+        const u32 w = (tot[word] >> shift) & mask;
+        __builtin_amdgcn_wave_barrier();
+        return w;
+    }
+};
+
+__global__ __launch_bounds__(256) void k4_pairs(const u32 *sidx, const u32 *jid_of, const PairRec *rec, const u64 *jkey, KeyFmt kf, const u32 *np,
+                                                 u32 *frag, int32_t *frag_j, u64 *head_mask, u64 *run_mask, const ContigStats *cs_chk, u64 *err_chk,
+                                                 int range_shift) {
+    __shared__ __attribute__((aligned(16))) u32 s_tot[4][16];
+    const u32 n = *np;
+    const int lane = lane_id();
+    const u32 wave = (u32)__builtin_amdgcn_readfirstlane((int)(threadIdx.x >> 6));
+    const u32 range = blockIdx.x * 4 + wave;
+    u32 *tot = s_tot[wave];
+    const FragWordOf word_of(lane);
+    const u64 first = (u64)range << (6 + range_shift);
+    if (first >= n) return;
+    const u32 i0 = (u32)first;
+    const u32 n_sl = min(1u << range_shift, (n - i0 + 63) >> 6);
+    auto at = [&](u32 s) { return min(i0 + 64u * s + (u32)lane, n - 1); };
+    auto key_of = [&](u32 jl) {
+        const u32 jf = (u32)__builtin_amdgcn_readfirstlane((int)jl);
+        return __ballot(jl != jf) == 0 ? jkey[jf] : jkey[jl];
+    };
+    u32 jv = jid_of[at(0)];
+    const u32 p0 = sidx[at(0)];
+    u32 j_nx = jid_of[at(1)], p_nx = sidx[at(1)];
+    u32 jprev_c = 0xffffffffu;
+    int32_t pos_c = 0, aend_c = 0;
+    if (i0 > 0) {
+        jprev_c = jid_of[i0 - 1];
+        const uint4 q = reinterpret_cast<const uint4 *>(rec + sidx[i0 - 1])[1];
+        pos_c = (int32_t)q.x;
+        aend_c = (int32_t)q.y;
+    }
+    PairRec Rc = rec_load(rec + p0);
+    u64 jk = key_of(jv);
+    u32 open_j = 0xffffffffu, fv = 0;
+    u64 fm = 0;
+    auto flush = [&]() {
+        if (open_j == 0xffffffffu) return;
+        const u32 slot = open_j + range;
+        if (lane < F_WORDS) frag[(size_t)slot * F_WORDS + lane] = lane == F_MISM_LO ? (u32)fm : lane == F_MISM_HI ? (u32)(fm >> 32) : fv;
+        if (lane == 0) frag_j[slot] = (int32_t)open_j;
+    };
+    auto absorb = [&](u32 jh, u32 w, u64 m64) {
+        if (jh != open_j) {
+            flush();
+            open_j = jh;
+            fv = w;
+            fm = m64;
+        } else {
+            fv = frag_combine(lane, fv, w);
+            fm += m64;
+        }
+    };
+    for (u32 s = 0; s < n_sl; s++) {
+        PairRec Rn = Rc;
+        u64 jkn = jk;
+        u32 j_n2 = j_nx, p_n2 = p_nx;
+        if (s + 1 < n_sl) {
+            Rn = rec_load(rec + p_nx);
+            jkn = key_of(j_nx);
+        }
+        if (s + 2 < n_sl) {
+            j_n2 = jid_of[at(s + 2)];
+            p_n2 = sidx[at(s + 2)];
+        }
+        const u32 i = i0 + 64u * s + (u32)lane;
+        const bool valid = i < n;
+#ifdef PJB_SELFCHECK
+        {
+            const u32 ic = valid ? i : n - 1;
+            const u32 Jc = cs_chk->J;
+            const u32 jb = ic ? jid_of[ic - 1] : jv;
+            int bad = 0;
+            if (sidx[ic] >= n) bad = 1;
+            else if (jv >= Jc) bad = 2;
+            else if (jv != jb && jv != jb + 1) bad = 3;
+            else if (ic == 0 && jv != 0) bad = 4;
+            else if (ic == n - 1 && jv != Jc - 1) bad = 5;
+            else if (frag_slot(jv, ic, range_shift) + 1 >= cs_chk->n_slots) bad = 6;
+            else if ((ic >> 6) >= cs_chk->n_slices) bad = 7;
+            else if (cs_chk->n_slots != frag_slots(Jc, n, range_shift)) bad = 8;
+            if (__ballot(bad != 0)) {
+                if (bad) set_error(err_chk, 0xffffe000u + (u32)bad, PJB_ERR_HIP);
+                return;
+            }
+        }
+#endif
+        u32 jprev_v = __shfl_up(jv, 1, 64);
+        int32_t pos_prev = __shfl_up(Rc.pos, 1, 64), aend_prev = __shfl_up(Rc.aend, 1, 64);
+        if (lane == 0) {
+            jprev_v = jprev_c;
+            pos_prev = pos_c;
+            aend_prev = aend_c;
+        }
+        u32 j = 0xffffffffu;
+        u32 cnt[4] = {0, 0, 0, 0}, jadp[5] = {0, 0, 0, 0, 0}, mx[5] = {0, 0, 0, 0, 0};
+        u32 first_mis = 100000000u;
+        u32 nb_mis = 0;
+        if (valid) {
+            j = jv;
+            int32_t istart, iend;
+            unpack_key(kf, jk, istart, iend);
+            const u64 rs = Rc.aux;
+            const u32 minMatch = (u32)(rs & 0xfffffu), mmes = (u32)((rs >> 20) & 0xfffffu), nbMis = (u32)(rs >> 40);
+            const u32 meta = Rc.meta;
+            const u32 cat = meta & META_CAT_MASK;
+            const u32 xs = (meta >> META_XS_SHIFT) & 3u;
+            const bool dist_head = i == 0 || jprev_v != j || pos_prev != Rc.pos || aend_prev != Rc.aend;
+            cnt[0] = 1u | ((u32)(cat == 0) << 8) | ((u32)(cat == 1) << 16) | ((u32)(cat == 2) << 24);
+            cnt[1] = (u32)(cat == 3) | ((u32)((meta & META_MULTI) != 0) << 8) | ((u32)(xs == 1) << 16) | ((u32)(xs == 2) << 24);
+            cnt[2] = (u32)((meta & META_UM) != 0) | ((u32)((meta & META_BPP) != 0) << 8) | ((u32)((meta & META_PPP) != 0) << 16) |
+                     ((u32)((meta & META_REL) != 0) << 24);
+            cnt[3] = (u32)dist_head;
+#pragma unroll
+            for (int w = 0; w < 5; w++)
+                jadp[w] = (u32)((u32)(4 * w) < minMatch) | ((u32)((u32)(4 * w + 1) < minMatch) << 8) |
+                          ((u32)((u32)(4 * w + 2) < minMatch) << 16) | ((u32)((u32)(4 * w + 3) < minMatch) << 24);
+            const int32_t la = istart - Rc.lstart, ra = Rc.rend - iend;
+            mx[0] = (u32)(la < ra ? la : ra);
+            mx[1] = Rc.updown & 0xffffu;
+            mx[2] = Rc.updown >> 16;
+            mx[3] = mmes;
+            mx[4] = minMatch;
+            first_mis = minMatch > 0 ? minMatch : 100000000u;
+            nb_mis = nbMis;
+            if (s == 0 && lane == 0) {
+                const int64_t u = frag_unused_before(j, i, jprev_v != j, range_shift);
+                if (u >= 0) frag_j[u] = -1;
+            }
+            const int64_t u = frag_unused_behind(j, i, n, range_shift);
+            if (u >= 0) frag_j[u] = -1;
+        }
+        const bool hj = valid && (i == 0 || jprev_v != j);
+        if (head_mask) {
+            const bool hr = valid && (hj || pos_prev != Rc.pos);
+            const u64 mj = __ballot(hj), mr = __ballot(hr);
+            if (lane == 0) {
+                head_mask[i >> 6] = mj;
+                run_mask[i >> 6] = mr;
+            }
+        }
+        jprev_c = (u32)__builtin_amdgcn_readlane((int)jv, 63);
+        pos_c = __builtin_amdgcn_readlane(Rc.pos, 63);
+        aend_c = __builtin_amdgcn_readlane(Rc.aend, 63);
+        u64 heads = __ballot(valid && (lane == 0 || jprev_v != j));
+        while (heads) {
+            const int h = __ffsll((unsigned long long)heads) - 1;
+            heads &= heads - 1;
+            const int e = heads ? __ffsll((unsigned long long)heads) - 1 : 64;
+            const bool in = lane >= h && lane < e;
+            const bool last = lane == 63;
+            auto add = [&](u32 v) { return wave_fold<DppAdd>(in ? v : 0u); };
+            auto top = [&](u32 v) { return wave_fold<DppMax>(in ? v : 0u); };
+            __builtin_amdgcn_wave_barrier();
+            FragWordOf::put(tot, FW_CNT / 4, last, add(cnt[0]), add(cnt[1]), add(cnt[2]), add(cnt[3]));
+            FragWordOf::put(tot, FW_MAX / 4, last, top(mx[0]), top(mx[1]), top(mx[2]), top(mx[3]));
+            FragWordOf::put(tot, 2, last, top(mx[4]), wave_fold<DppMin>(in ? first_mis : 100000000u), add(jadp[0]), add(jadp[1]));
+            FragWordOf::put(tot, 3, last, add(jadp[2]), add(jadp[3]), add(jadp[4]), 0u);
+            const u32 mis = wave_total<DppAdd>(in ? nb_mis : 0u);
+            absorb((u32)__builtin_amdgcn_readlane((int)j, h), word_of.get(tot), (u64)mis);
+        }
+        Rc = Rn;
+        jk = jkn;
+        jv = j_nx;
+        j_nx = j_n2;
+        p_nx = p_n2;
+    }
+    flush();
+}
+
 constexpr int FRAG_SLOTS_PER_WAVE = 16;
 __global__ __launch_bounds__(256) void k5_frag_reduce(const u32 *frag, const int32_t *frag_j, const u32 *n_slots_p, u32 *acc) {
     const u32 n_slots = *n_slots_p;
```

New measurement: 31.51 billion reads/s, median of 6. 1.05x the previous value.
